# USTC-StarTeam/DR4SR

Hardware: AMD Instinct MI355X
Metric: training sequences/sec, SASRec d=64 L=50 (higher is better)
Workload: dtype f32; 1 GPU; SASRec on amazon-toys-shaped synthetic rows (BASELINE configs[1]): N=11925, L=50, d=64, 2 layers, 2 heads, FFN 128, dropout 0.50, B=256 rows/GPU/step, toys histogram (10.9% valid) seqlen; global_batch=256, seq_len=50, parallelism=dp1, hip_graph=True, steps_per_graph=30

## Files before the change

dr4sr_amd/_lib.py:

```python
from __future__ import annotations

import ctypes as C
import os

_HERE = os.path.dirname(os.path.abspath(__file__))
LIB_PATH = os.environ.get("DR4SR_LIB_PATH") or os.path.join(_HERE, "csrc", "libdr4sr_hip.so")

ABI_VERSION = 10
COMM_ID_BYTES = 128
GRAD_TAIL = 4
STATE_WORDS = 16
STATE_STEP, STATE_T, STATE_NVALID, STATE_RNGSTEP = 0, 1, 2, 3
POOL_NONE, POOL_ORIGIN, POOL_LAST, POOL_MEAN = 0, 1, 2, 3
SITE_EMB, SITE_ATTN, SITE_PROJ, SITE_ACT, SITE_FFN = 0, 1, 2, 3, 4
OPT_ADAM, OPT_SGD, OPT_ADAGRAD, OPT_RMSPROP = 0, 1, 2, 3


def check_ids(idx, n_items: int, what: str = "index"):
    import torch
    if idx is None or idx.numel() == 0:
        return
    bad = torch.zeros(1, dtype=torch.int32, device=idx.device)
    t = idx.contiguous()
    check(load().dr4sr_check_ids(ptr(t), t.numel(), int(n_items), ptr(bad), cur_stream()), "dr4sr_check_ids")
# ... 21 lines not shown
    if n == "rmsprop":
        return OPT_RMSPROP, (0.9, 0.99), 1e-8, float(weight_decay)
    if n == "sparse_adam":
        raise RuntimeError("SparseAdam does not support dense gradients, please consider Adam instead")
    return OPT_ADAM, (0.9, 0.999), 1e-8, 0.0

KERNEL_IDS = {"prep": 0, "embed_fwd": 1, "qkv_fwd": 2, "attn_fwd": 3, "post_fwd": 4, "score": 5, "transpose": 6,
              "post_bwd": 7, "attn_bwd": 8, "qkv_bwd": 9, "embed_bwd": 10, "wgrad": 11, "adam": 12, "zero_grads": 13,
              "embqkv_fwd": 14, "post_mid": 15, "qkv_embed_bwd": 16, "wgrad_fused": 17}

FMLP_KERNEL_IDS = {"filter_fwd": 0, "ffn_fwd": 1, "ffn_bwd": 2, "filter_bwd": 3, "wgrad": 4}

_f32p = C.c_void_p
_i64p = C.c_void_p


_PLAN_BUFFERS = [("seed", C.c_uint64),
                 ("params", _f32p), ("grads", _f32p), ("adam_m", _f32p), ("adam_v", _f32p),
                 ("n_params", C.c_int64)]
_PLAN_WORKSPACE = [("sample_neg", C.c_int32),
                   ("workspace", C.c_void_p), ("workspace_bytes", C.c_int64),
                   ("state", C.c_void_p)]
_PLAN_OPTIMIZER = [("lr", C.c_float), ("beta1", C.c_float), ("beta2", C.c_float), ("adam_eps", C.c_float), ("weight_decay", C.c_float)]
_PLAN_PERM_LOG = [("perm", _i64p), ("n_perm", C.c_int64), ("perm_stride", C.c_int64), ("perm_offset", C.c_int64),
                  ("perm_counter", C.c_void_p),
                  ("loss_log", _f32p)]


def _i32(*names):
    return [(n, C.c_int32) for n in names]


def _ptrs(*names):
    return [(n, _i64p) for n in names]


class SasrecPlan(C.Structure):
    _fields_ = (_i32("abi_version", "B", "L", "D", "H", "F", "n_layer", "n_items") + [("ln_eps", C.c_float), ("p_drop", C.c_float)]
                + _PLAN_BUFFERS + _ptrs("in_item_id", "item_id", "seqlen", "rows", "neg_item") + _PLAN_WORKSPACE + _PLAN_OPTIMIZER
                + _PLAN_PERM_LOG + _i32("expected_tokens", "optimizer"))


class MetaWeighting(C.Structure):
    _fields_ = [("phi", _f32p), ("gumbel", _f32p), ("user_id", _i64p), ("gate_in", C.c_void_p), ("gate_out", C.c_void_p),
                ("weight_out", _f32p), ("tau", C.c_float)]


class FmlpPlan(C.Structure):
    _fields_ = (_i32("abi_version", "B", "L", "D", "F", "n_layer", "n_items") + [("ln_eps", C.c_float), ("p_drop", C.c_float)]
                + _PLAN_BUFFERS + _ptrs("in_item_id", "item_id", "rows", "neg_item") + _PLAN_WORKSPACE + _PLAN_OPTIMIZER
                + _i32("optimizer") + _PLAN_PERM_LOG)


class GruPlan(C.Structure):
    _fields_ = (_i32("abi_version", "B", "L", "D", "H", "n_layer", "n_items") + [("p_drop", C.c_float)]
                + _PLAN_BUFFERS + _ptrs("in_item_id", "item_id", "seqlen", "rows", "neg_item") + _PLAN_WORKSPACE + _PLAN_OPTIMIZER
                + _i32("optimizer") + _PLAN_PERM_LOG)


class RegenPlan(C.Structure):
    _fields_ = [
        ("abi_version", C.c_int32),
        ("n_rows", C.c_int32), ("K", C.c_int32), ("max_len", C.c_int32),
        ("D", C.c_int32), ("H", C.c_int32), ("F", C.c_int32), ("n_layer", C.c_int32),
        ("ln_eps", C.c_float),
        ("params", _f32p),
        ("n_params", C.c_int64),
    ]


REGEN_TENSORS = 70
REGEN_SCORE_TENSORS = 98

_PLANP = C.POINTER(SasrecPlan)
_FPLANP = C.POINTER(FmlpPlan)
_GPLANP = C.POINTER(GruPlan)
_RPLANP = C.POINTER(RegenPlan)

SYMBOLS = {
    "dr4sr_abi_version": (C.c_int, []),
    "dr4sr_sasrec_plan_sizeof": (C.c_int, []),
    "dr4sr_sasrec_param_layout": (C.c_int64, [C.c_int32, C.c_int32, C.c_int32, C.c_int32, C.c_int32, C.c_void_p]),
    "dr4sr_sasrec_workspace_bytes": (C.c_int64, [_PLANP]),
    "dr4sr_sasrec_at_scale": (C.c_int, [C.c_void_p]),
    "dr4sr_sasrec_fwd_bwd": (C.c_int, [_PLANP, C.c_void_p]),
    "dr4sr_adam_step": (C.c_int, [_PLANP, C.c_void_p]),
    "dr4sr_sasrec_fwd_bwd_weighted": (C.c_int, [_PLANP, C.c_void_p, C.c_void_p]),
    "dr4sr_sasrec_fwd_bwd_weighted_prepared": (C.c_int, [_PLANP, C.c_void_p, C.c_void_p]),
    "dr4sr_sasrec_train_step": (C.c_int, [_PLANP, C.c_void_p]),
    "dr4sr_sasrec_train_steps": (C.c_int, [_PLANP, C.c_int32, C.c_void_p]),
    "dr4sr_sasrec_fwd_bwd_prepared": (C.c_int, [_PLANP, C.c_void_p]),
    "dr4sr_adam_step_prepare_next": (C.c_int, [_PLANP, C.c_void_p]),
    "dr4sr_sasrec_grad_buckets": (C.c_int, [_PLANP, C.POINTER(C.c_int64)]),
    "dr4sr_sasrec_fwd_bwd_phase": (C.c_int, [_PLANP, C.c_int32, C.c_int32, C.c_void_p]),
    "dr4sr_sasrec_encode": (C.c_int, [_PLANP, C.c_int32, C.c_int32, _f32p, C.c_void_p]),
    "dr4sr_sasrec_encode_bwd": (C.c_int, [_PLANP, C.c_int32, C.c_int32, _f32p, C.c_void_p]),
    "dr4sr_select_rows": (C.c_int, [_i64p, C.c_int64, _i64p, C.c_int32, C.c_int64, C.c_int64, C.c_void_p, C.c_void_p]),
    "dr4sr_embed_gather_posadd": (C.c_int, [_f32p, _f32p, _i64p, _f32p, C.c_int64, C.c_int32, C.c_int32, C.c_int32, C.c_void_p]),
    "dr4sr_score_bce_fwd": (C.c_int, [_f32p, _f32p, _i64p, _i64p, _f32p, _f32p, _f32p, _f32p, C.c_int64, C.c_int32, C.c_int32, C.c_void_p]),
    "dr4sr_score_bce_bwd": (C.c_int, [_f32p, _f32p, _i64p, _i64p, _f32p, _f32p, _f32p, _f32p, C.c_int64, C.c_int32, C.c_int32, C.c_void_p]),
    "dr4sr_score_bpr_fwd": (C.c_int, [_f32p, _f32p, _i64p, _i64p, _f32p, _f32p, _f32p, _f32p, C.c_int64, C.c_int32, C.c_int32, C.c_void_p]),
    "dr4sr_score_bpr_bwd": (C.c_int, [_f32p, _f32p, _i64p, _i64p, _f32p, _f32p, _f32p, _f32p, C.c_int64, C.c_int32, C.c_int32, C.c_void_p]),
    "dr4sr_loss_from_scores_fwd": (C.c_int, [_f32p, _f32p, C.c_int64, C.c_int32, C.c_int32, _f32p, _f32p, C.c_void_p]),
    "dr4sr_loss_from_scores_bwd": (C.c_int, [_f32p, _f32p, C.c_int64, C.c_int32, C.c_int32, _f32p, _f32p, _f32p, _f32p, C.c_void_p]),
    "dr4sr_neg_sample": (C.c_int, [_i64p, C.c_int64, C.c_int32, C.c_uint64, C.c_uint32, C.c_void_p]),
    "dr4sr_neg_sample_dev": (C.c_int, [_i64p, C.c_int64, C.c_int32, C.c_uint64, C.c_void_p, C.c_void_p]),
    "dr4sr_dropout_mask": (C.c_int, [_f32p, C.c_int64, C.c_float, C.c_uint64, C.c_uint32, C.c_uint32, C.c_void_p]),
    "dr4sr_fmlp_plan_sizeof": (C.c_int, []),
    "dr4sr_fmlp_param_layout": (C.c_int64, [C.c_int32, C.c_int32, C.c_int32, C.c_int32, C.c_int32, C.c_void_p]),
    "dr4sr_fmlp_workspace_bytes": (C.c_int64, [_FPLANP]),
    "dr4sr_fmlp_fwd_bwd": (C.c_int, [_FPLANP, C.c_void_p]),
    "dr4sr_fmlp_train_step": (C.c_int, [_FPLANP, C.c_void_p]),
    "dr4sr_fmlp_encode": (C.c_int, [_FPLANP, C.c_int32, _f32p, C.c_void_p]),
    "dr4sr_fmlp_encode_bwd": (C.c_int, [_FPLANP, C.c_int32, _f32p, C.c_void_p]),
    "dr4sr_gru4rec_plan_sizeof": (C.c_int, []),
    "dr4sr_gru4rec_param_layout": (C.c_int64, [C.c_int32, C.c_int32, C.c_int32, C.c_int32, C.c_void_p]),
    "dr4sr_gru4rec_workspace_bytes": (C.c_int64, [_GPLANP]),
    "dr4sr_gru4rec_uses_cooperative": (C.c_int, [C.c_int32, C.c_int32]),
    "dr4sr_gru4rec_uses_wavefront": (C.c_int, [C.c_int32, C.c_int32, C.c_int32, C.c_int32]),
    "dr4sr_gru4rec_fwd_bwd": (C.c_int, [_GPLANP, C.c_void_p]),
    "dr4sr_gru4rec_train_step": (C.c_int, [_GPLANP, C.c_void_p]),
    "dr4sr_gru4rec_encode": (C.c_int, [_GPLANP, C.c_int32, C.c_int32, _f32p, C.c_void_p]),
    "dr4sr_gru4rec_encode_bwd": (C.c_int, [_GPLANP, C.c_int32, C.c_int32, _f32p, C.c_void_p]),
    "dr4sr_adam_flat": (C.c_int, [_f32p, _f32p, _f32p, _f32p, C.c_int64, C.c_void_p, C.c_float, C.c_float, C.c_float, C.c_float, C.c_float, C.c_void_p]),
    "dr4sr_reload_env": (C.c_int, []),
    "dr4sr_build_flags": (C.c_int, []),
    "dr4sr_sasrec_launch_kernel": (C.c_int, [_PLANP, C.c_int32, C.c_int32, C.c_void_p]),
    "dr4sr_sasrec_launch_kernel_weighted": (C.c_int, [_PLANP, C.c_void_p, C.c_int32, C.c_int32, C.c_void_p]),
    "dr4sr_gru4rec_launch_kernel": (C.c_int, [_GPLANP, C.c_int32, C.c_int32, C.c_void_p]),
    "dr4sr_fmlp_launch_kernel": (C.c_int, [_FPLANP, C.c_int32, C.c_int32, C.c_void_p]),
    "dr4sr_meta_param_count": (C.c_int64, [C.c_int32]),
    "dr4sr_meta_select_workspace_floats": (C.c_int64, [C.c_int64]),
    "dr4sr_meta_select_workspace_floats_d": (C.c_int64, [C.c_int64, C.c_int32]),
    "dr4sr_meta_select_fwd": (C.c_int, [_f32p, _f32p, _f32p, C.c_uint64, C.c_uint32, C.c_void_p, C.c_float, _i64p, _i64p, C.c_int64, C.c_int32,
                                        C.c_int32, C.c_void_p, C.c_void_p, _f32p, C.c_void_p]),
    "dr4sr_meta_select_bwd": (C.c_int, [_f32p, _f32p, _f32p, C.c_uint64, C.c_uint32, C.c_void_p, C.c_float, _i64p, _i64p, C.c_int64, C.c_int32,
                                        C.c_int32, C.c_void_p, _f32p, _f32p, _f32p, _f32p, _f32p, C.c_void_p]),
    "dr4sr_meta_select_fwd_d": (C.c_int, [_f32p, _f32p, _f32p, C.c_uint64, C.c_uint32, C.c_void_p, C.c_float, _i64p, _i64p, C.c_int64, C.c_int32,
                                          C.c_int32, C.c_void_p, C.c_void_p, _f32p, C.c_void_p]),
    "dr4sr_meta_select_bwd_d": (C.c_int, [_f32p, _f32p, _f32p, C.c_uint64, C.c_uint32, C.c_void_p, C.c_float, _i64p, _i64p, C.c_int64, C.c_int32,
                                          C.c_int32, C.c_void_p, _f32p, _f32p, _f32p, _f32p, _f32p, C.c_void_p]),
    "dr4sr_fd_step_size": (C.c_int, [_f32p, _f32p, C.c_int64, C.c_float, _f32p, C.c_void_p]),
    "dr4sr_fd_step_size_scratch_floats": (C.c_int64, []),
    "dr4sr_fd_step_size_ws": (C.c_int, [_f32p, _f32p, C.c_int64, C.c_float, _f32p, _f32p, C.c_void_p]),
    "dr4sr_fd_shift": (C.c_int, [_f32p, _f32p, _f32p, _f32p, C.c_float, C.c_int64, C.c_void_p]),
    "dr4sr_fd_neumann": (C.c_int, [_f32p, _f32p, _f32p, _f32p, _f32p, _f32p, _f32p, C.c_float, C.c_int64, C.c_void_p]),
    "dr4sr_fd_diff": (C.c_int, [_f32p, _f32p, _f32p, _f32p, _f32p, _f32p, C.c_float, C.c_int64, C.c_void_p]),
    "dr4sr_fd_diff4": (C.c_int, [_f32p, _f32p, _f32p, _f32p, _f32p, _f32p, _f32p, C.c_float, C.c_int64, C.c_void_p]),
    "dr4sr_scale_by": (C.c_int, [_f32p, _f32p, _f32p, C.c_int64, C.c_void_p]),
    "dr4sr_meta_opt_step": (C.c_int, [C.c_int32, _f32p, _f32p, _f32p, _f32p, C.c_int32, C.c_float, C.c_float, C.c_float, C.c_float, C.c_float,
                                      C.c_float, C.c_void_p, _f32p, C.c_void_p]),
    "dr4sr_meta_sgd_step": (C.c_int, [_f32p, _f32p, _f32p, C.c_int32, C.c_float, C.c_float, C.c_float, C.c_float, C.c_void_p,
                                      _f32p, C.c_void_p]),
    "dr4sr_cl_augment": (C.c_int, [_i64p, _i64p, _i64p, _i64p, C.c_int32, C.c_int32, C.c_int32, C.c_double, C.c_double, C.c_double,
                                   C.c_int64, C.c_uint64, C.c_uint32, C.c_void_p]),
    "dr4sr_cl_augment_dev": (C.c_int, [_i64p, _i64p, _i64p, _i64p, C.c_int32, C.c_int32, C.c_int32, C.c_double, C.c_double, C.c_double,
                                       C.c_int64, C.c_uint64, C.c_void_p, C.c_uint32, C.c_void_p]),
    "dr4sr_cl_augment2_dev": (C.c_int, [_i64p, _i64p, _i64p, _i64p, _i64p, _i64p, C.c_int32, C.c_int32, C.c_int32, C.c_double, C.c_double,
                                        C.c_double, C.c_int64, C.c_uint64, C.c_void_p, C.c_uint32, C.c_void_p]),
    "dr4sr_cl_augment2_rows_dev": (C.c_int, [_i64p, _i64p, _i64p, _i64p, _i64p, _i64p, _i64p, C.c_int32, C.c_int32, C.c_int32, C.c_double,
                                             C.c_double, C.c_double, C.c_int64, C.c_uint64, C.c_void_p, C.c_uint32, C.c_void_p]),
    "dr4sr_cl_prepare": (C.c_int, [_i64p, C.c_int32, C.c_void_p, _f32p, _f32p, C.c_int64, C.c_void_p]),
    "dr4sr_cl_prepare_rows": (C.c_int, [_i64p, _i64p, C.c_int32, C.c_void_p, _f32p, _f32p, C.c_int64, C.c_void_p]),
    "dr4sr_cl_prepare_rows_step": (C.c_int, [_i64p, _i64p, C.c_int32, C.c_void_p, _f32p, _f32p, C.c_int64, C.c_void_p, C.c_int32, C.c_void_p]),
    "dr4sr_infonce_bwd_scaled": (C.c_int, [_f32p, _f32p, C.c_void_p, C.c_int32, C.c_int32, C.c_float, _f32p, _f32p, _f32p, C.c_float, C.c_int32,
                                           _f32p, _f32p, C.c_void_p]),
# ... 125 lines not shown
```

dr4sr_amd/csrc/attn_tile.h:

```cpp
#pragma once
#include "common.h"
#include "kernels.h"

#define TSTAMP(i, thr) do { if (P.stamps && blockIdx.x == 0 && threadIdx.x == (thr)) P.stamps[i] = __builtin_amdgcn_s_memtime(); } while (0)
namespace tattn {

constexpr int WR = 80;
constexpr int QR0 = 64;
constexpr int MT = WR / 16;

template <int D>
struct Lds {
    static constexpr int LD = D + 4;
    static constexpr int floats = 2 * WR * LD + 16 * LD + 64 + 32 + 2 * WR + 8;
    float *Kw, *Vw, *Qs, *st, *rd; int2* tok; unsigned* pad;
    __device__ __forceinline__ explicit Lds(float* base) {
        Kw = base; Vw = Kw + WR * LD; Qs = Vw + WR * LD;
        st = Qs + 16 * LD;
        rd = st + 64;
        tok = reinterpret_cast<int2*>(rd + 32);
        pad = reinterpret_cast<unsigned*>(tok + WR);
    }
};

// ... 53 lines not shown
    __device__ __forceinline__ void issue(const TileAttnArgs& A, const int t0, const int T, const int r_lo = 0, const int r_hi = WR) {
        const int wb = t0 - QR0, lo = max(0, t0 - (A.L - 1)), hi = min(T, t0 + 16);
        tw = make_int2(0x7fffffff, 0);
        if ((int)threadIdx.x >= r_lo && (int)threadIdx.x < r_hi) {
            const int tk = wb + (int)threadIdx.x;
            if (tk >= lo && tk < hi) tw = A.tok[tk];
        }
#pragma unroll
        for (int q = 0; q < PER; ++q) {
            const int f = threadIdx.x + 256 * q, r = f / C4, c4 = f % C4, tk = wb + r;
            v[q] = make_float4(0.f, 0.f, 0.f, 0.f);
            if (r >= r_lo && r < r_hi && tk >= lo && tk < hi) v[q] = ld4(A.qkv + (size_t)tk * 3 * D + D + 4 * c4);
        }
        if constexpr (WITH_Q) {
#pragma unroll
            for (int q = 0; q < QPER; ++q) {
                const int f = threadIdx.x + 256 * q, r = f / (D / 4), c4 = f % (D / 4);
                qv[q] = make_float4(0.f, 0.f, 0.f, 0.f);
                if (t0 + r < T) qv[q] = ld4(A.qkv + (size_t)(t0 + r) * 3 * D + 4 * c4);
            }
        }
        sv = make_float2(0.f, 0.f);
        if constexpr (WITH_STAT) {
            if (threadIdx.x < 32) {
                const int i = threadIdx.x >> 1;
                if (t0 + i < T) sv = *reinterpret_cast<const float2*>(A.stat + ((size_t)(t0 + i) * 2 + (threadIdx.x & 1)) * 2);
            }
        }
    }
    __device__ __forceinline__ void commit(const Lds<D>& S, const int r_lo = 0, const int r_hi = WR) const {
        if ((int)threadIdx.x >= r_lo && (int)threadIdx.x < r_hi) S.tok[threadIdx.x] = tw;
        if (threadIdx.x < 128) {
            const unsigned long long bal = __ballot(((tw.y >> 30) & 1) != 0);
            if (threadIdx.x == 0) {
#pragma unroll
                for (int jt = 0; jt < 4; ++jt)
                    if (16 * jt >= r_lo && 16 * jt < r_hi) S.pad[jt] = (unsigned)(bal >> (16 * jt)) & 0xffffu;
            }
            if (threadIdx.x == 64 && 64 >= r_lo && 64 < r_hi) S.pad[4] = (unsigned)bal & 0xffffu;
        }
#pragma unroll
        for (int q = 0; q < PER; ++q) {
            const int f = threadIdx.x + 256 * q, r = f / C4, c4 = f % C4;
            if (r >= r_lo && r < r_hi) st4((4 * c4 < D ? S.Kw + r * LD + 4 * c4 : S.Vw + r * LD + 4 * c4 - D), v[q]);
        }
        if constexpr (WITH_Q) {
#pragma unroll
            for (int q = 0; q < QPER; ++q) {
                const int f = threadIdx.x + 256 * q, r = f / (D / 4), c4 = f % (D / 4);
                st4(S.Qs + r * LD + 4 * c4, qv[q]);
            }
        }
        if constexpr (WITH_STAT) {
            if (threadIdx.x < 32) {
                const int i = threadIdx.x >> 1, h = threadIdx.x & 1;
                S.st[(h * 16 + i) * 2] = sv.x; S.st[(h * 16 + i) * 2 + 1] = sv.y;
            }
        }
    }
};

constexpr int NEAR0 = WR - 32;
template <int D>
__device__ __forceinline__ void far_rows_if_needed(const TileAttnArgs& A, const Lds<D>& S, const int t0, const int T) {
    if (!(A.on & 4) || S.tok[QR0].x >= t0 - 16) return;
    Stage<D, false, false> st;
    st.issue(A, t0, T, 0, NEAR0);
    st.commit(S, 0, NEAR0);
    lds_barrier();
}

struct Keep { uint32_t lo, hi; };
__device__ __forceinline__ int2 own_word(const TileAttnArgs& A, const int t0, const int T) {
    const int tq = t0 + (int)(threadIdx.x & 15);
    return tq < T ? A.tok[tq] : make_int2(0x7fffffff, 0);
}
__device__ __forceinline__ Keep own_keep(const PostArgs& P, const int2 mq, const int t0, const int T) {
    Keep k{0xffffffffu, 0xffffffffu};
    if (P.training && P.p > 0.f) {
        const int tq = t0 + (int)(threadIdx.x & 15), h = (threadIdx.x >> 6) & 1, i = tq < T ? tq - mq.x : -1;
        const RngKey rk = make_rng(P.seed, (uint32_t)P.state[DR4SR_STATE_RNGSTEP], P.p);
        keep_bits(rk, DR4SR_SITE_ATTN + 4 * P.layer, ((uint64_t)((mq.y & 0xfffff) * 2 + h) * 64 + i) * 64, i, k.lo, k.hi);
    }
    return k;
}

template <int D, bool KEEP_QS>
struct FwdPre { Stage<D, KEEP_QS, false> st; int2 mq_g; float qf[D / 8]; uint32_t klo, khi; };
template <int D, bool KEEP_QS>
__device__ __forceinline__ void fwd_issue(const PostArgs& P, const int t0, const int T, FwdPre<D, KEEP_QS>& F) {
    constexpr int DH = D / 2;
    const TileAttnArgs& A = P.at;
    const int h = (threadIdx.x >> 6) & 1;
    F.mq_g = own_word(A, t0, T);
    if constexpr (!KEEP_QS) frag_g<DH>(F.qf, A.qkv + h * DH, 3 * D, t0, T);
    F.st.issue(A, t0, T, (A.on & 4) ? NEAR0 : 0, WR);
}
template <int D, bool KEEP_QS>
__device__ __forceinline__ void fwd_stage(const PostArgs& P, const int t0, const int T, float* base, FwdPre<D, KEEP_QS>& F) {
    const TileAttnArgs& A = P.at;
    const Lds<D> S(base);
    const int r_lo = (A.on & 4) ? NEAR0 : 0;
    TSTAMP(27, 0);
    __builtin_amdgcn_sched_barrier(0);
    const Keep k0 = own_keep(P, F.mq_g, t0, T);
    F.klo = k0.lo; F.khi = k0.hi;
    __builtin_amdgcn_sched_barrier(0);
    TSTAMP(28, 0);
    F.st.commit(S, r_lo, WR);
    TSTAMP(8, 0);
    lds_barrier();
    far_rows_if_needed<D>(A, S, t0, T);
    TSTAMP(9, 0);
}
template <int D, bool KEEP_QS>
__device__ __forceinline__ Keep fwd_compute(const PostArgs& P, const int t0, const int T, float* R0, const int ldr, float* base, FwdPre<D, KEEP_QS>& F) {
    constexpr int DH = D / 2, LD = D + 4, H = 2;
    const TileAttnArgs& A = P.at;
    const Lds<D> S(base);
    const int lane = threadIdx.x & 63, w = threadIdx.x >> 6, h = w & 1, half = w >> 1, i16 = lane & 15, g = lane >> 4;
    const uint32_t klo_ = F.klo, khi_ = F.khi;
    float qf[DH / 4];
    if constexpr (!KEEP_QS) {
#pragma unroll
        for (int c = 0; c < DH / 4; ++c) qf[c] = F.qf[c];
    }
    if constexpr (KEEP_QS) frag<DH>(qf, S.Qs, LD, 0, h * DH);
    const int tq = t0 + i16, wb = t0 - QR0;
    const int2 mq = S.tok[QR0 + i16];
    const bool qok = tq < T;
    const int qs = mq.x;
    const int jt_lo = (S.tok[QR0].x - wb) >> 4;
    const float scale = 1.0f / sqrtf((float)DH);
    f32x4 s[MT];
    float m = -INFINITY;
#pragma unroll
    for (int jt = 0; jt < MT; ++jt) {
        s[jt] = (f32x4){0.f, 0.f, 0.f, 0.f};
        if (jt >= jt_lo) {
            float kf[DH / 4];
            frag<DH>(kf, S.Kw, LD, jt * 16, h * DH);
            s[jt] = mma_rows<DH>(kf, qf);
            const unsigned pw = S.pad[jt] >> (4 * g);
#pragma unroll
            for (int r = 0; r < 4; ++r) {
                const int tk = wb + jt * 16 + 4 * g + r;
                const bool ok = qok && tk >= qs && tk <= tq && !((pw >> r) & 1u);
                const float v = ok ? s[jt][r] * scale : -INFINITY;
                s[jt][r] = v;
                m = fmaxf(m, v);
            }
        }
    }
    TSTAMP(10, 0);
    m = xg_max(m);
    float sum = 0.f;
#pragma unroll
    for (int jt = 0; jt < MT; ++jt)
        if (jt >= jt_lo)
#pragma unroll
            for (int r = 0; r < 4; ++r) { const float e = __expf(s[jt][r] - m); s[jt][r] = e; sum += e; }
    sum = xg_sum(sum);
    const float inv = 1.0f / sum;
    if (half == 0 && g == 0) {
        if (qok) { float* st = A.stat + ((size_t)tq * H + h) * 2; st[0] = m; st[1] = inv; }
        if constexpr (KEEP_QS) { S.st[(h * 16 + i16) * 2] = m; S.st[(h * 16 + i16) * 2 + 1] = inv; }
// ... 154 lines not shown
```

dr4sr_amd/csrc/embed.hip:

```cpp
#include "common.h"
#include "kernels.h"
#include <cstdlib>

template <int D>
__global__ __launch_bounds__(256) void k_embed_dense(const float* __restrict__ E, const float* __restrict__ P,
                                                         const int64_t* __restrict__ idx, float* __restrict__ out,
                                                         int64_t ntok, int L, int n_items) {
    constexpr int LPT = D / 4;
    constexpr int TPB = 256 / LPT;
    const int sub = threadIdx.x / LPT, c = (threadIdx.x % LPT) * 4;
    for (int64_t t = (int64_t)blockIdx.x * TPB + sub; t < ntok; t += (int64_t)gridDim.x * TPB) {
        int64_t id = idx[t];
        id = id < 0 ? 0 : (id >= n_items ? n_items - 1 : id);
        const int l = (int)(t % L);
        const float4 e = ld4(E + id * D + c);
        const float4 p = ld4(P + (size_t)l * D + c);
        const f32x4 v = {e.x + p.x, e.y + p.y, e.z + p.z, e.w + p.w};
        __builtin_nontemporal_store(v, reinterpret_cast<f32x4*>(out + t * D + c));
    }
}

extern "C" int dr4sr_embed_gather_posadd(const float* E, const float* P, const int64_t* idx, float* out,
                                         int64_t B, int32_t L, int32_t D, int32_t n_items, void* stream) {
    if (!E || !P || !idx || !out || B < 0 || L <= 0 || n_items <= 0) return DR4SR_E_ARG;
    if (D != 64 && D != 128) return DR4SR_E_SHAPE;
    const int64_t ntok = B * L;
    if (ntok == 0) return 0;
    const int tpb = 256 / (D / 4);
    int64_t blocks = (ntok + tpb - 1) / tpb;
    const int64_t cap = DR4SR_XENV("DR4SR_GATHER_BLOCKS") ? atoll(DR4SR_XENV("DR4SR_GATHER_BLOCKS")) : 65536;
    if (blocks > cap) blocks = cap;
    hipStream_t s = (hipStream_t)stream;
    if (D == 64) hipLaunchKernelGGL(k_embed_dense<64>, dim3((unsigned)blocks), dim3(256), 0, s, E, P, idx, out, ntok, L, n_items);
    else hipLaunchKernelGGL(k_embed_dense<128>, dim3((unsigned)blocks), dim3(256), 0, s, E, P, idx, out, ntok, L, n_items);
    return DR4SR_LAUNCH_CHECK();
}

__global__ __launch_bounds__(256) void k_check_ids(const int64_t* __restrict__ idx, int64_t n, int n_items, int* __restrict__ bad) {
    int c = 0;
    for (int64_t i = (int64_t)blockIdx.x * 256 + threadIdx.x; i < n; i += (int64_t)gridDim.x * 256) {
        const int64_t id = idx[i];
        c += (id < 0 || id >= n_items) ? 1 : 0;
    }
    c = (int)wave_sum((float)c);
    if ((threadIdx.x & 63) == 0 && c) atomicAdd(bad, c);
}
extern "C" int dr4sr_check_ids(const int64_t* idx, int64_t n, int32_t n_items, int32_t* bad_count, void* stream) {
    if (!idx || !bad_count || n < 0 || n_items <= 0) return DR4SR_E_ARG;
    if (n == 0) return 0;
    int64_t blocks = (n + 255) / 256;
    if (blocks > 1024) blocks = 1024;
    hipLaunchKernelGGL(k_check_ids, dim3((unsigned)blocks), dim3(256), 0, (hipStream_t)stream, idx, n, n_items, bad_count);
    return DR4SR_LAUNCH_CHECK();
}

#include "prep_body.h"
__global__ __launch_bounds__(1024) void k_prep(const PrepArgs P, float* __restrict__ zero, int64_t zero_n4) {
    if (blockIdx.x > 0) {
        for (int64_t i = (int64_t)(blockIdx.x - 1) * 1024 + threadIdx.x; i < zero_n4; i += (int64_t)(gridDim.x - 1) * 1024)
            st4(zero + 4 * i, make_float4(0.f, 0.f, 0.f, 0.f));
        return;
    }
    __shared__ unsigned long long part[1024];
    prep_body<1024>(P, part);
}

static int launch_prep_sel(const int64_t* seqlen, const int64_t* rows, int* cu, int* state, int B, int L, int bump_rng, float* zero,
                           int64_t zero_floats, const PermSel& sel, int* tile_seq, int* seq_class, hipStream_t s) {
    const int64_t n4 = zero ? zero_floats / 4 : 0;
    int zb = (int)((n4 + 1023) / 1024);
    if (zb > 255) zb = 255;
    const PrepArgs P{seqlen, rows, cu, state, B, L, bump_rng, sel, tile_seq, seq_class, nullptr};
    hipLaunchKernelGGL(k_prep, dim3(1 + zb), dim3(1024), 0, s, P, zero, n4);
    return DR4SR_LAUNCH_CHECK();
}
int launch_prep_raw(const int64_t* seqlen, const int64_t* rows, int* cu, int* state, int B, int L, int bump_rng, float* zero,
                    int64_t zero_floats, hipStream_t s) {
    return launch_prep_sel(seqlen, rows, cu, state, B, L, bump_rng, zero, zero_floats, PermSel{nullptr, 0, 0, 0, nullptr}, nullptr, nullptr, s);
}
int launch_prep_raw_hints(const int64_t* seqlen, const int64_t* rows, int* cu, int* state, int B, int L, int bump_rng, float* zero,
                          int64_t zero_floats, int* tile_seq, const PermSel& sel, hipStream_t s) {
    return launch_prep_sel(seqlen, rows, cu, state, B, L, bump_rng, zero, zero_floats, sel, tile_seq, nullptr, s);
}
int make_prep_args(const dr4sr_sasrec_plan* p, const Workspace& ws, int bump_rng, PrepArgs* out) {
    PermSel sel{nullptr, 0, 0, 0, nullptr};
    if (p->perm && bump_rng) {
        if (!p->rows || !p->perm_counter || p->n_perm <= 0) return DR4SR_E_ARG;
        sel = PermSel{p->perm, p->n_perm, p->perm_stride, p->perm_offset, p->perm_counter};
    }
    *out = PrepArgs{p->seqlen, p->rows, ws.cu, p->state, p->B, p->L, bump_rng, sel, ws.tile_seq, (ws.attn_split && !attn_wave_on(p, ws)) ? ws.seq_class : nullptr, ws.len_buf};
    return 0;
}
int launch_prep(const dr4sr_sasrec_plan* p, const Workspace& ws, int bump_rng, int zero_grads, hipStream_t s) {
    PrepArgs P;
    const int rc = make_prep_args(p, ws, bump_rng, &P);
    if (rc) return rc;
    return launch_prep_sel(p->seqlen, p->rows, ws.cu, p->state, p->B, p->L, bump_rng, zero_grads ? p->grads : nullptr,
                           ws.n_params + DR4SR_GRAD_TAIL, P.sel, ws.tile_seq, P.seq_class, s);
}


template <int D>
__global__ __launch_bounds__(256) void k_embed_fwd(const float* __restrict__ E, const float* __restrict__ P,
                                                   const int64_t* __restrict__ idx, const int64_t* __restrict__ rows,
                                                   const int* __restrict__ cu, float* __restrict__ X, int B, int L,
                                                   int n_items, const int* __restrict__ state, uint64_t seed, float p,
                                                   int training) {
    constexpr int LPT = D / 4, TPB = 256 / LPT;
    const int T = state[DR4SR_STATE_T];
    const int t = blockIdx.x * TPB + threadIdx.x / LPT, c = (threadIdx.x % LPT) * 4;
    if (t >= T) return;
    const int b = find_seq(cu, B, t), pos = t - cu[b];
    const int64_t row = rows ? rows[b] : b;
    int64_t id = idx[row * L + pos];
    id = id < 0 ? 0 : (id >= n_items ? n_items - 1 : id);
    float4 o = ld4(E + id * D + c);
    if (P) {
        const float4 pe = ld4(P + (size_t)pos * D + c);
        o = make_float4(o.x + pe.x, o.y + pe.y, o.z + pe.z, o.w + pe.w);
    }
    if (training && p > 0.f) {
        const RngKey rk = make_rng(seed, (uint32_t)state[DR4SR_STATE_RNGSTEP], p);
        const float4 m = drop4(rk, DR4SR_SITE_EMB, ((uint64_t)b * L + pos) * D + c);
        o.x *= m.x; o.y *= m.y; o.z *= m.z; o.w *= m.w;
    }
    st4(X + (size_t)t * D + c, o);
}

int launch_embed_fwd_raw(const float* E, const float* P, const int64_t* idx, const int64_t* rows, const int* cu, float* X, int B,
                         int L, int D, int n_items, const int* state, uint64_t seed, float p, int training, hipStream_t s) {
    dim3 grid(((int64_t)B * L + (256 / (D / 4)) - 1) / (256 / (D / 4))), blk(256);
    if (D == 64) hipLaunchKernelGGL(k_embed_fwd<64>, grid, blk, 0, s, E, P, idx, rows, cu, X, B, L, n_items, state, seed, p, training);
    else hipLaunchKernelGGL(k_embed_fwd<128>, grid, blk, 0, s, E, P, idx, rows, cu, X, B, L, n_items, state, seed, p, training);
    return DR4SR_LAUNCH_CHECK();
}
int launch_embed_fwd(const dr4sr_sasrec_plan* p, const Workspace& ws, int training, hipStream_t s) {
    return launch_embed_fwd_raw(p->params + ws.off[0], p->params + ws.off[1], p->in_item_id, p->rows, ws.cu, ws.X[0], p->B, p->L,
                                p->D, p->n_items, p->state, p->seed, p->p_drop, training, s);
}

template <int D>
__global__ __launch_bounds__(256) void k_embed_bwd(const float* __restrict__ dX, const int64_t* __restrict__ idx,
                                                   const int64_t* __restrict__ rows, const int* __restrict__ cu,
                                                   float* __restrict__ dE, float* __restrict__ dP, int B, int L,
                                                   int n_items, const int* __restrict__ state, uint64_t seed, float p,
                                                   int training) {
    constexpr int LPT = D / 4, TPB = 256 / LPT;
    __shared__ float accP[64 * D];
    const int T = state[DR4SR_STATE_T], t0 = blockIdx.x * 64;
    if (t0 >= T) return;
    if (dP) for (int i = threadIdx.x; i < L * D; i += 256) accP[i] = 0.f;
    __syncthreads();
    const int c = (threadIdx.x % LPT) * 4;
    const bool dodrop = training && p > 0.f;
    const RngKey rk = make_rng(seed, (uint32_t)state[DR4SR_STATE_RNGSTEP], p);
    for (int t = t0 + threadIdx.x / LPT; t < min(T, t0 + 64); t += TPB) {
        const int b = find_seq(cu, B, t), pos = t - cu[b];
        const int64_t row = rows ? rows[b] : b;
        float4 g = ld4(dX + (size_t)t * D + c);
        if (dodrop) {
            const float4 m = drop4(rk, DR4SR_SITE_EMB, ((uint64_t)b * L + pos) * D + c);
            g.x *= m.x; g.y *= m.y; g.z *= m.z; g.w *= m.w;
        }
        if (dP) {
            float* a = accP + pos * D + c;
            atomicAdd(a, g.x); atomicAdd(a + 1, g.y); atomicAdd(a + 2, g.z); atomicAdd(a + 3, g.w);
        }
        const int64_t id = idx[row * L + pos];
        if (id > 0 && id < n_items) {
            float* d = dE + id * D + c;
            unsafeAtomicAdd(d, g.x); unsafeAtomicAdd(d + 1, g.y); unsafeAtomicAdd(d + 2, g.z); unsafeAtomicAdd(d + 3, g.w);
        }
    }
    if (dP) {
        __syncthreads();
        for (int i = threadIdx.x; i < L * D; i += 256) {
            const float v = accP[i];
            if (v != 0.f) unsafeAtomicAdd(dP + i, v);
        }
    }
}
// ... 127 lines not shown
```

dr4sr_amd/csrc/kernels.h:

```cpp
#pragma once
#include <hip/hip_runtime.h>
#include <stdint.h>
#include "../../include/dr4sr_hip.h"
#include "../../include/dr4sr_hip_hooks.h"
#include "prep_body.h"

#define DR4SR_MAX_LAYERS 8

struct LayerWs {
    float* qkv;
    float* ctx;
    float* attn_st;
    unsigned* attn_keep;
    float* u1;
    float* y;
    float* st1;
    float* a;
    float* h;
    float* u2;
    float* st2;
    float* df;
    float* da;
    float* du1;
    float* dout;
    float* dqkv;
    unsigned short* row_keep;
};

struct Workspace {
    int64_t off[2 + 12 * DR4SR_MAX_LAYERS];
    int64_t n_params;
    int Tmax;
    int* cu;
    bool scale, attn_split;
    bool attn_tile_sa;
    int* len_buf;
    int* seq_class;
    float* attn_rd;
    int* tile_seq;
    float* X[DR4SR_MAX_LAYERS + 1];
    float* dX[DR4SR_MAX_LAYERS + 1];
    float* dctx;
    int4* de_rec;
    int* idx32;
    int2* tok;
    int4* de_ent;
    unsigned char* de_off;
    bool det;
    bool scale_wg, det_lat; float* det_kv; int64_t det_kv_layer;
    float* det_part; float* det_ln; float* det_dp; int64_t det_stride;
    float* wfrag;
    unsigned short* wsplit;
    int64_t wsplit_E;
    float* wT;
    int64_t wT_stride;
    float* score_part;
    float* ln_part;
    LayerWs layer[DR4SR_MAX_LAYERS];
    int64_t bytes;
};

enum { P_IN_W = 0, P_IN_B, P_OUT_W, P_OUT_B, P_W1, P_B1, P_W2, P_B2, P_LN1_W, P_LN1_B, P_LN2_W, P_LN2_B };
static inline int64_t poff(const Workspace& ws, int layer, int j) { return ws.off[2 + 12 * layer + j]; }
int latency_tmax();
static inline bool at_scale(int Tmax) { return Tmax > latency_tmax(); }
constexpr int DR4SR_SCALE_TOKENS = 7168, DR4SR_ATTN_SPLIT_TOKENS = 14336;
constexpr int DR4SR_SCALE_TOKENS_SHORT = 10240, DR4SR_SCALE_TOKENS_LONG = 6144;
constexpr int DR4SR_SCALE_TOKENS_SHORT_WAVE = 7680;
bool attn_tile_capable(const dr4sr_sasrec_plan* p);
bool tile_xcd_order(const dr4sr_sasrec_plan* p, const Workspace& ws);
__host__ __device__ inline int xcd_per(const int tiles, const int BM) {
    const int q = BM < 64 ? 64 / BM : 1, per = (tiles + 7) >> 3;
    return (per + q - 1) / q * q;
}
static inline int xcd_grid(int tiles, int BM) { return 8 * xcd_per(tiles, BM); }
#if defined(__HIPCC__)
__device__ __forceinline__ int xcd_tile(const int T, const int BM, const int on) {
    if (!on) return (int)blockIdx.x;
    const int nt = (T + BM - 1) / BM, per = xcd_per(nt, BM), x = (int)blockIdx.x & 7, j = (int)blockIdx.x >> 3;
    return (j < per && x * per + j < nt) ? x * per + j : nt;
}
#endif

struct TileAttnArgs {
    const float* qkv; float* dqkv; float* ctx; float* stat; const int2* tok; int L;
    unsigned* keep;
    int on;
    float* kv_part;
};
struct alignas(16) PostArgs {
    const float* ctx; const float* x;
    const float* out_w; const float* out_b; const float* ln1_w; const float* ln1_b;
    const float* w1; const float* b1; const float* w2; const float* b2; const float* ln2_w; const float* ln2_b;
    float* u1; float* y; float* st1; float* a; float* h; float* u2; float* st2; float* z;
    const float* dz; const float* w2T; const float* w1T; const float* out_wT;
    float* df; float* da; float* du1; float* dout; float* dctx;
    float* rd; int n_head;
    float* ln_part;
    const int* state; uint64_t seed; float p; float eps; int layer; int training;
    uint32_t sP, sA, sF;
    unsigned long long* stamps;
    const float* nx_in_w; const float* nx_in_b; float* nx_qkv;
    const float* up_dqkv; const float* up_in_w; const float* up_du1;
    const float* up_kv_part;
    TileAttnArgs at;
    int xcd;
    float* nx_dqkv_zero;
    float* dn_dqkv_zero;
    int wt_attn;
    unsigned short* row_keep;
    const unsigned short* sp;
};

struct EmbQkvArgs {
    const float* E; const float* P; const int64_t* idx; const int64_t* rows; const int* cu; const int* tile_seq; float* X;
    const float* W; const float* bias; float* QKV; const int* state;
    int B, L, n_items, training; uint64_t seed; float p;
    int* idx32;
    int2* tok; float* dqkv_zero;
    int xcd;
    int wf_layers;
    const unsigned short* sp;
};
struct QkvEmbBwdArgs {
    const float* dQKV; const float* W; const float* dU1; const int64_t* idx; const int64_t* rows; const int* cu; const int* tile_seq;
    float* dE; float* dP; const int* state; int B, L, n_items, training; uint64_t seed; float p;
    float* gout;
    const float* kv_part; const int2* tok;
    const unsigned short* sp;
};

struct ScoreTileArgs {
    const float* E; float* dE; const int64_t* target; const int64_t* rows; const int* cu; const int* tile_seq; int64_t* neg_item; float* part;
    int sample_neg, n_items, B, L;
    int4* rec;
    int4* ent; unsigned char* off; const int* idx32; int logG;
    const float* phi; const float* gumbel; const int64_t* user_id; const unsigned long long* gate_in; unsigned long long* gate_out;
    float* w_out; float inv_tau; uint64_t meta_seed;
};

struct WgradJob {
    const float* G; int ldg; int gcol;
    const float* X; int ldx;
    float* dW; float* db;
    int ldw;
};
#define DR4SR_DET_MAX_SPLITS 320
#define DR4SR_WGRAD_MAX_JOBS 12
struct WgradArgs {
    WgradJob job[DR4SR_WGRAD_MAX_JOBS * DR4SR_MAX_LAYERS];
    int jobs_per_layer;
    const int* state; uint64_t seed; float p; int training;
    const float* ln_part; int64_t ln_layer_stride; float* grads; int64_t o_ln1_w; int64_t layer_stride;
    const float* score_part; float* tail; int B; int D;
    int score_tiles;
    int ln_tile_rows;
    int ln_rows[DR4SR_MAX_LAYERS];
    int qeb_plane;
    int layer0;
    int bf16x3;
    int xcd;
    const float* fc_dm; int64_t fc_o_cw; int fc_L;
    const float* sc_g; const int64_t* sc_idx; const int64_t* sc_rows; const int* sc_tile_seq; const int* cu;
    float* sc_dE; float* sc_dP; int sc_L; int sc_n_items;
    const int4* ow_ent; const unsigned char* ow_off;
    int ow_on; const int4* ow_rec; const int* ow_idx32; const float* ow_z; int ow_logG, ow_planes, ow_rpo;
    float* det; int det_stride; float* det_ln; float* det_dp;
};

bool wave_tiles(const dr4sr_sasrec_plan* p, const Workspace& ws);
bool wt_bwd_on();
int launch_wt_post_fwd(const PostArgs& A, int Tmax, hipStream_t s);
int launch_wt_post_bwd(const PostArgs& A, int Tmax, hipStream_t s);

int launch_wt_post_mid(const PostArgs& A, const ScoreTileArgs& S, int Tmax, hipStream_t s);
int launch_wt_embqkv_fwd(const EmbQkvArgs& A, int Tmax, hipStream_t s);
int launch_wt_qkv_embed_bwd(const QkvEmbBwdArgs& A, int Tmax, hipStream_t s);

int ffn_tile_rows(int Tmax);
int launch_ffn_fwd(const PostArgs& A, int Tmax, hipStream_t s);
int launch_ffn_bwd(const PostArgs& A, int Tmax, hipStream_t s);
int launch_fmlp_wgrad(const WgradArgs& A, int Tmax, int n_layer, hipStream_t s);
int launch_table_owner64(const int* state, const int4* rec, const int* idx32, const float* z, const float* g, float* dE, int n_items, hipStream_t s);
int launch_adam_flat(float* P, float* G, float* M, float* V, int64_t n, int* state, float lr, float b1, float b2, float eps, float wd, hipStream_t s,
                     float* loss_log = nullptr, const int* log_index = nullptr, const PrepArgs* next = nullptr, int opt = DR4SR_OPT_ADAM);

int carve_workspace(const dr4sr_sasrec_plan* p, Workspace* ws);

int launch_prep(const dr4sr_sasrec_plan* p, const Workspace& ws, int bump_rng, int zero_grads, hipStream_t s);
int make_prep_args(const dr4sr_sasrec_plan* p, const Workspace& ws, int bump_rng, PrepArgs* out);
int launch_embed_fwd(const dr4sr_sasrec_plan* p, const Workspace& ws, int training, hipStream_t s);
int launch_embed_bwd(const dr4sr_sasrec_plan* p, const Workspace& ws, int training, hipStream_t s);
int launch_unpack(const dr4sr_sasrec_plan* p, const Workspace& ws, const float* X, float* out, int mode, hipStream_t s);
int launch_pack(const dr4sr_sasrec_plan* p, const Workspace& ws, const float* dout, float* dX, int mode, hipStream_t s);

int launch_transpose_weights(const dr4sr_sasrec_plan* p, const Workspace& ws, hipStream_t s);
bool tile_bf3(const dr4sr_sasrec_plan* p, const Workspace& ws);
int launch_wsplit(const dr4sr_sasrec_plan* p, const Workspace& ws, hipStream_t s);
int launch_wfrag_write(const dr4sr_sasrec_plan* p, const Workspace& ws, hipStream_t s);
bool wfrag_img_on(const dr4sr_sasrec_plan* p, const Workspace& ws);
int launch_wsplit_raw(const float* params, unsigned short* img, int64_t o_in, int64_t o_out, int64_t o_w1, int64_t o_w2, int64_t layer_stride,
                      int E, int D, int F, int n_layer, hipStream_t s);
int launch_embqkv_fwd(const dr4sr_sasrec_plan* p, const Workspace& ws, int training, hipStream_t s);
int launch_qkv_embed_bwd(const dr4sr_sasrec_plan* p, const Workspace& ws, int training, hipStream_t s);
int launch_post_mid(const dr4sr_sasrec_plan* p, const Workspace& ws, int training, hipStream_t s, const dr4sr_meta_weighting* mw = nullptr);
int launch_qkv_fwd(const dr4sr_sasrec_plan* p, const Workspace& ws, int layer, hipStream_t s);
int launch_post_fwd(const dr4sr_sasrec_plan* p, const Workspace& ws, int layer, int training, hipStream_t s);
int launch_post_bwd(const dr4sr_sasrec_plan* p, const Workspace& ws, int layer, int training, hipStream_t s);
int launch_qkv_bwd(const dr4sr_sasrec_plan* p, const Workspace& ws, int layer, hipStream_t s);
int launch_wgrad(const dr4sr_sasrec_plan* p, const Workspace& ws, int training, int with_score, hipStream_t s, bool qeb = false,
                 bool meta = false, int l_lo = 0, int l_hi = -1, int table = -1);
bool wgrad_table_jobs(const dr4sr_sasrec_plan* p, const Workspace& ws);
bool attn_in_tile(const dr4sr_sasrec_plan* p, const Workspace& ws);
bool attn_wave_on(const dr4sr_sasrec_plan* p, const Workspace& ws);
bool attn_fold_fwd(const dr4sr_sasrec_plan* p, const Workspace& ws);
PostArgs make_post_args(const dr4sr_sasrec_plan* p, const Workspace& ws, int layer, int training);
int launch_attn_tile_fwd(const dr4sr_sasrec_plan* p, const Workspace& ws, int layer, int training, hipStream_t s);
int launch_attn_tile_bwd(const dr4sr_sasrec_plan* p, const Workspace& ws, int layer, int training, hipStream_t s);
bool qeb_in_wgrad(const Workspace& ws);

int launch_attn_fwd(const dr4sr_sasrec_plan* p, const Workspace& ws, int layer, int training, hipStream_t s);
int launch_attn_bwd(const dr4sr_sasrec_plan* p, const Workspace& ws, int layer, int training, hipStream_t s);

struct GruWaveArgs {
    const float* gi1; const float* whh[2]; const float* wih2; const int* cu;
    float* r[2]; float* z[2]; float* n[2]; float* ghn[2]; float* hprev[2]; float* hout[2];
    const float* dhout; float* dgi[2]; float* dgh[2];
};
int launch_prep_raw(const int64_t* seqlen, const int64_t* rows, int* cu, int* state, int B, int L, int bump_rng, float* zero,
                    int64_t zero_floats, hipStream_t s);
int launch_prep_raw_hints(const int64_t* seqlen, const int64_t* rows, int* cu, int* state, int B, int L, int bump_rng, float* zero,
                          int64_t zero_floats, int* tile_seq, const PermSel& sel, hipStream_t s);
int launch_embed_fwd_raw(const float* E, const float* P, const int64_t* idx, const int64_t* rows, const int* cu, float* X, int B,
                         int L, int D, int n_items, const int* state, uint64_t seed, float p, int training, hipStream_t s);
int launch_embed_bwd_raw(const float* dX, const int64_t* idx, const int64_t* rows, const int* cu, float* dE, float* dP, int B, int L,
                         int D, int n_items, const int* state, uint64_t seed, float p, int training, hipStream_t s);
int launch_unpack_raw(const float* X, const int* cu, float* out, int B, int L, int D, int last, hipStream_t s);
int launch_pack_raw(const float* dout, const int* cu, float* dX, int B, int L, int D, int last, hipStream_t s);
int launch_score_packed_raw(const float* Z, const float* E, float* dE, float* dZ, const int64_t* target, const int64_t* rows,
                            const int* cu, int64_t* neg_item, int sample_neg, float* part, const int* state, uint64_t seed,
                            int n_items, int B, int L, int D, hipStream_t s, int4* rec = nullptr);

int launch_attn2_fwd(const dr4sr_sasrec_plan* p, const Workspace& ws, int layer, int training, hipStream_t s);
int launch_attn2_bwd(const dr4sr_sasrec_plan* p, const Workspace& ws, int layer, int training, hipStream_t s);

int launch_score_packed(const dr4sr_sasrec_plan* p, const Workspace& ws, hipStream_t s);
int launch_adam(const dr4sr_sasrec_plan* p, hipStream_t s, const PrepArgs* next = nullptr);
```

dr4sr_amd/csrc/linear.hip:

```cpp
#include "common.h"
#include "kernels.h"
#include <cstdlib>
#define STAMP(i) do { if (A.stamps && blockIdx.x == 0 && threadIdx.x == 0) A.stamps[i] = __builtin_amdgcn_s_memtime(); } while (0)

extern __shared__ __attribute__((aligned(16))) float smem[];

__global__ __launch_bounds__(256) void k_transpose(const float* __restrict__ params, float* __restrict__ wT,
                                                   int64_t o_in, int64_t o_out, int64_t o_w1, int64_t o_w2,
                                                   int64_t layer_stride, int64_t wT_stride, int D, int F) {
    const int m = blockIdx.y, layer = blockIdx.z;
    const float* src;
    float* dst = wT + layer * wT_stride;
    int R, C;
    if (m == 0) { src = params + o_in + layer * layer_stride; R = 3 * D; C = D; }
    else if (m == 1) { src = params + o_out + layer * layer_stride; R = D; C = D; dst += 3 * D * D; }
    else if (m == 2) { src = params + o_w1 + layer * layer_stride; R = F; C = D; dst += 4 * D * D; }
    else { src = params + o_w2 + layer * layer_stride; R = D; C = F; dst += 4 * D * D + D * F; }
    for (int i = blockIdx.x * 256 + threadIdx.x; i < R * C; i += gridDim.x * 256) {
        const int r = i / C, c = i % C;
        dst[c * R + r] = src[i];
    }
}

int launch_transpose_weights(const dr4sr_sasrec_plan* p, const Workspace& ws, hipStream_t s) {
// ... 187 lines not shown
template <int BM, int D>
__global__ __launch_bounds__(256) void k_embqkv_fwd(const EmbQkvArgs A) {
    constexpr int N = 3 * D, LDA = D + 4, LPT = D / 4, TPB = 256 / LPT;
    if constexpr (BM == 16 && D == 128) { if (A.wf_layers > 0) wfrag_image_write<D>(A); }
    const int T = A.state[DR4SR_STATE_T], t0 = xcd_tile(T, BM, A.xcd) * BM;
    if (t0 >= T) return;
    float* As = smem;
    const int c = (threadIdx.x % LPT) * 4;
    const bool dodrop = A.training && A.p > 0.f;
    const RngKey rk = make_rng(A.seed, (uint32_t)A.state[DR4SR_STATE_RNGSTEP], A.p);
    constexpr bool PFE = BM == 16 && D == 64;
    WFragT<PFE ? D : 16, PFE ? N : 64> f_in;
    if constexpr (PFE) wfrag_load(f_in, A.W, D);
    const int bh = A.tile_seq[t0 >> 4];
#pragma unroll
    for (int r0 = 0; r0 < BM; r0 += TPB) {
        const int r = r0 + threadIdx.x / LPT, t = t0 + r;
        if (r < BM) {
            float4 o = make_float4(0.f, 0.f, 0.f, 0.f);
            if (t < T) {
                const int b = find_seq_from(A.cu, A.B, t, bh), pos = t - A.cu[b];
                const int64_t row = A.rows ? A.rows[b] : b;
                int64_t id = A.idx[row * A.L + pos];
                if (A.idx32 && c == 0) A.idx32[t] = (id > 0 && id < A.n_items) ? (int)id : 0;
                if (A.tok && c == 0) A.tok[t] = make_int2(t - pos, b | ((A.cu[b + 1] - A.cu[b]) << 20) | (id == 0 ? 1 << 30 : 0));
                id = id < 0 ? 0 : (id >= A.n_items ? A.n_items - 1 : id);
                o = ld4(A.E + id * D + c);
                const float4 pe = ld4(A.P + (size_t)pos * D + c);
                o = make_float4(o.x + pe.x, o.y + pe.y, o.z + pe.z, o.w + pe.w);
                if (dodrop) {
                    const float4 m = drop4(rk, DR4SR_SITE_EMB, ((uint64_t)b * A.L + pos) * D + c);
                    o.x *= m.x; o.y *= m.y; o.z *= m.z; o.w *= m.w;
                }
                st4(A.X + (size_t)t * D + c, o);
            }
            st4(As + r * LDA + c, o);
        }
    }
    lds_barrier();
    TileAcc<BM, N> acc;
    tile_zero(acc);
    if constexpr (PFE) tile_mma_frag<BM, D, N>(As, LDA, f_in, acc);
    else tile_gemm<D == 128 && BM == 32, BM, D, N>(As, LDA, A.W, D, false, A.sp, WSplitGeo<D, 128>::E, 0, acc);
    tile_to_global<BM, N>(acc, A.QKV, N, A.bias, t0, T);
    if (A.dqkv_zero) zero_kv_rows<BM, D>(A.dqkv_zero, t0, T);
}

int launch_embqkv_fwd(const dr4sr_sasrec_plan* p, const Workspace& ws, int training, hipStream_t s) {
    const int D = p->D, bm = tile_rows(ws);
    const size_t lds = sizeof(float) * bm * (D + 4);
    dim3 grid((ws.Tmax + bm - 1) / bm), blk(256);
    EmbQkvArgs A;
    A.E = p->params + ws.off[0]; A.P = p->params + ws.off[1]; A.idx = p->in_item_id; A.rows = p->rows; A.cu = ws.cu; A.tile_seq = ws.tile_seq; A.X = ws.X[0];
    A.W = p->params + poff(ws, 0, P_IN_W); A.bias = p->params + poff(ws, 0, P_IN_B); A.QKV = ws.layer[0].qkv; A.state = p->state;
    A.B = p->B; A.L = p->L; A.n_items = p->n_items; A.training = training; A.seed = p->seed; A.p = p->p_drop;
    A.idx32 = de_owner_mode(ws) ? ws.idx32 : nullptr;
    A.sp = wsplit_of(p, ws, 0); A.wf_layers = 0;
    if (wfrag_img_on(p, ws)) { A.sp = reinterpret_cast<const unsigned short*>(ws.wfrag); A.wf_layers = p->n_layer; }
    const bool in_tile = attn_in_tile(p, ws);
    A.tok = (in_tile || ws.attn_tile_sa || attn_wave_on(p, ws)) ? ws.tok : nullptr; A.dqkv_zero = in_tile ? ws.layer[0].dqkv : nullptr;
    A.xcd = tile_xcd_order(p, ws) ? 1 : 0;
    if (A.xcd) grid.x = xcd_grid((int)grid.x, bm);
    if (wave_tiles(p, ws)) return launch_wt_embqkv_fwd(A, ws.Tmax, s);
#define EQ(B_) do { if (D == 64) hipLaunchKernelGGL((k_embqkv_fwd<B_, 64>), grid, blk, lds, s, A); \
                    else hipLaunchKernelGGL((k_embqkv_fwd<B_, 128>), grid, blk, lds, s, A); } while (0)
    BM_DISPATCH(bm, EQ);
#undef EQ
    return DR4SR_LAUNCH_CHECK();
}


struct LnCarry { float4 v; float mean, rstd; uint32_t keep; };
template <int F>
struct RowCarry { LnCarry ln1, ln2; float4 a[F / 64]; uint32_t akeep; };
__host__ __device__ constexpr bool carry_vals(int CARRY) { return CARRY != 0; }
__host__ __device__ constexpr bool carry_bits(int CARRY) { return CARRY == 1 || CARRY == 3; }
__device__ __forceinline__ uint32_t keep_bits4(const float4& m) {
    return (m.x != 0.f ? 1u : 0u) | (m.y != 0.f ? 2u : 0u) | (m.z != 0.f ? 4u : 0u) | (m.w != 0.f ? 8u : 0u);
}
__device__ __forceinline__ float4 keep_factors4(const RngKey& k, uint32_t bits) {
    return make_float4((bits & 1u) ? k.scale : 0.f, (bits & 2u) ? k.scale : 0.f, (bits & 4u) ? k.scale : 0.f, (bits & 8u) ? k.scale : 0.f);
}

template <int BM, int D, bool RES_IN_LDS, bool COPY_LDS, bool CARRY = false, bool KPRE = false>
__device__ __forceinline__ void ln_rowpass(const float* __restrict__ Cs, int ldc, const float* res, int ldres,
                                           const float* __restrict__ lnw, const float* __restrict__ lnb, float eps,
                                           float* __restrict__ U, float* __restrict__ OUT, float* __restrict__ ST,
                                           float* Ls, int ldl, int t0, int T, bool dodrop, const RngKey& rk,
                                           uint32_t site, float4 (*yreg)[D / 64] = nullptr, LnCarry* cy = nullptr) {
    constexpr int NV = D / 64, PASSES = BM / 16;
    static_assert(!CARRY || (NV == 1 && PASSES == 1), "the carried row state is one float4 per thread");
    static_assert(!KPRE || CARRY, "the keep bits arrive in the carried row state");
    const int l16 = threadIdx.x & 15, rsub = threadIdx.x >> 4;
    float4 gam[NV], bet[NV], v[PASSES][NV];
    float mean[PASSES], rstd[PASSES];
#pragma unroll
    for (int j = 0; j < NV; ++j) { gam[j] = ld4(lnw + 4 * l16 + 64 * j); bet[j] = ld4(lnb + 4 * l16 + 64 * j); }
#pragma unroll
    for (int ps = 0; ps < PASSES; ++ps) {
        const int row = ps * 16 + rsub, t = t0 + row;
        const bool ok = t < T;
#pragma unroll
        for (int j = 0; j < NV; ++j) {
            const int c = 4 * l16 + 64 * j;
            float4 o = ld4(Cs + row * ldc + c);
            float4 r = make_float4(0.f, 0.f, 0.f, 0.f);
            if (RES_IN_LDS) r = ld4(res + row * ldres + c);
            else if constexpr (KPRE) r = cy->v;
            else if (ok) r = ld4(res + (size_t)t * ldres + c);
            if (dodrop) {
                float4 m;
                if constexpr (KPRE) m = keep_factors4(rk, cy->keep); else m = drop4(rk, site, (uint64_t)t * D + c);
                o.x *= m.x; o.y *= m.y; o.z *= m.z; o.w *= m.w;
                if constexpr (CARRY && !KPRE) cy->keep = keep_bits4(m);
            }
            v[ps][j] = make_float4(r.x + o.x, r.y + o.y, r.z + o.z, r.w + o.w);
            if (ok) st4(U + (size_t)t * D + c, v[ps][j]);
        }
    }
#pragma unroll
    for (int ps = 0; ps < PASSES; ++ps) ln_stats16<NV>(v[ps], mean[ps], rstd[ps], eps);
    if constexpr (CARRY) { cy->v = v[0][0]; cy->mean = mean[0]; cy->rstd = rstd[0]; }
#pragma unroll
    for (int ps = 0; ps < PASSES; ++ps) {
        const int row = ps * 16 + rsub, t = t0 + row;
        const bool ok = t < T;
#pragma unroll
        for (int j = 0; j < NV; ++j) {
            const int c = 4 * l16 + 64 * j;
            const float m = mean[ps], rs = rstd[ps];
            const float4 yv = make_float4((v[ps][j].x - m) * rs * gam[j].x + bet[j].x, (v[ps][j].y - m) * rs * gam[j].y + bet[j].y,
                                          (v[ps][j].z - m) * rs * gam[j].z + bet[j].z, (v[ps][j].w - m) * rs * gam[j].w + bet[j].w);
            if (ok && OUT) st4(OUT + (size_t)t * D + c, yv);
            if (yreg) yreg[ps][j] = ok ? yv : make_float4(0.f, 0.f, 0.f, 0.f);
            if (COPY_LDS) st4(Ls + row * ldl + c, ok ? yv : make_float4(0.f, 0.f, 0.f, 0.f));
        }
        if (ok && l16 == 0) { ST[2 * (size_t)t] = mean[ps]; ST[2 * (size_t)t + 1] = rstd[ps]; }
    }
}

template <int F>
__device__ __forceinline__ void row_keep_store(const PostArgs& A, const RowCarry<F>& cy, const int t0, const int T) {
    static_assert(F == 128, "16 bits per thread");
    const int t = t0 + (threadIdx.x >> 4);
    if (t < T) A.row_keep[16 * (size_t)t + (threadIdx.x & 15)] = (unsigned short)(cy.ln1.keep | (cy.ln2.keep << 4) | (cy.akeep << 8));
}
__device__ __forceinline__ uint32_t row_keep_word(const RngKey& rk, const uint32_t sP, const uint32_t sF, const uint32_t sA, const bool actdrop, const int t) {
    constexpr int D = 64, F = 128;
    const int l16 = threadIdx.x & 15, pr = l16 >> 1;
    const bool odd = l16 & 1;
    const uint32_t b0 = drop_bits8(rk, odd ? sF : sP, (uint64_t)t * D + 8 * pr);
    const uint32_t b1 = actdrop ? drop_bits8(rk, sA, (uint64_t)t * F + (odd ? 64 : 0) + 8 * pr) : 0xffu;
    const uint32_t own0 = odd ? b0 >> 4 : b0 & 15u, own1 = odd ? b1 >> 4 : b1 & 15u;
    const uint32_t give = odd ? (b0 & 15u) | ((b1 & 15u) << 4) : (b0 >> 4) | (b1 & 0xf0u);
    const uint32_t got = (uint32_t)__shfl_xor((int)give, 1, 64), got0 = got & 15u, got1 = got >> 4;
    return odd ? got0 | (own0 << 4) | (got1 << 8) | (own1 << 12) : own0 | (got0 << 4) | (own1 << 8) | (got1 << 12);
}
template <int BM, int D, int F, bool FFN_ONLY, bool KEEPQ = false, int CARRY = 0, bool KU = false>
__device__ __forceinline__ void post_fwd_body(const PostArgs& A, const int t0, const int T, float4 (*zreg)[D / 64] = nullptr,
                                              tattn::Keep* keep_out = nullptr, RowCarry<F>* cy = nullptr) {
    constexpr int LD = D + 4, LF = F + 4, NVF = F / 64, PASSES = BM / 16;
    float* R0 = smem;
    float* R1 = R0 + BM * LD;
    float* R2 = R1 + BM * LD;
    const int l16 = threadIdx.x & 15, rsub = threadIdx.x >> 4;
    const bool dodrop = A.training && A.p > 0.f;
    const RngKey rk = make_rng(A.seed, (uint32_t)A.state[DR4SR_STATE_RNGSTEP], A.p);
    const uint32_t sP = A.sP, sA = A.sA, sF = A.sF;
    const bool actdrop = dodrop && sA != 0xffffffffu;

    constexpr bool PF = BM == 16 && !FFN_ONLY;
    WFragT<PF ? D : 16, PF ? D : 64> f_out;
    WFragT<PF ? D : 16, PF ? F : 64> f_w1;
    WFragT<PF ? F : 16, PF ? D : 64> f_w2;
    WFragT<PF ? D : 16, PF ? 3 * D : 64> f_nx;
    STAMP(0);
    static_assert(!KU || (BM == 16 && D == 64 && F == 128 && !FFN_ONLY && CARRY != 0), "one row, one float4, 16 keep bits per thread");
    auto keep_upfront = [&]() {
        if constexpr (KU) {
            const uint32_t w = row_keep_word(rk, sP, sF, sA, actdrop, t0 + rsub);
            cy->ln1.keep = w & 15u; cy->ln2.keep = (w >> 4) & 15u; cy->akeep = w >> 8;
        }
    };
    if constexpr (KU) {
        const int t = t0 + rsub;
        cy->ln1.v = t < T ? ld4(A.x + (size_t)t * D + 4 * l16) : make_float4(0.f, 0.f, 0.f, 0.f);
        __builtin_amdgcn_sched_barrier(0);
    }
    if (FFN_ONLY) {
        load_tile_bm<BM, D>(R1, LD, A.x, D, t0, T);
    } else {
        constexpr bool AT = BM == 16 && (D == 64 || D == 128);
        bool at_on = false;
        if constexpr (AT) at_on = A.at.on != 0;
        if (!at_on) load_tile_bm<BM, D>(R0, LD, A.ctx, D, t0, T);
        tattn::FwdPre<AT ? D : 64, KEEPQ> att_pre;
#ifdef DR4SR_WFRAG_UPFRONT
        constexpr bool SPREAD = false;
#else
        constexpr bool SPREAD = AT && PF;
#endif
        constexpr bool KU_EARLY = KU && SPREAD;
        if constexpr (SPREAD) {
            if (at_on) {
                tattn::fwd_issue<D, KEEPQ>(A, t0, T, att_pre);
                __builtin_amdgcn_sched_barrier(0);
                { if constexpr (D == 128) wfrag_load_img(f_out, reinterpret_cast<const float*>(A.sp) + WSplitGeo<D, F>::OUT); else wfrag_load(f_out, A.out_w, D); }
                __builtin_amdgcn_sched_barrier(0);
                if constexpr (KU_EARLY) { keep_upfront(); __builtin_amdgcn_sched_barrier(0); }
                tattn::fwd_stage<D, KEEPQ>(A, t0, T, smem + att_lds_off(D, F), att_pre);
                __builtin_amdgcn_sched_barrier(0);
                { if constexpr (D == 128) wfrag_load_img(f_w1, reinterpret_cast<const float*>(A.sp) + WSplitGeo<D, F>::W1); else wfrag_load(f_w1, A.w1, D); }
                { if constexpr (D == 128) wfrag_load_img(f_w2, reinterpret_cast<const float*>(A.sp) + WSplitGeo<D, F>::W2); else wfrag_load(f_w2, A.w2, F); }
                __builtin_amdgcn_sched_barrier(0);
                const tattn::Keep k = tattn::fwd_compute<D, KEEPQ>(A, t0, T, R0, LD, smem + att_lds_off(D, F), att_pre);
                if (keep_out) *keep_out = k;
                __builtin_amdgcn_sched_barrier(0);
                if (A.nx_qkv) { if constexpr (D == 128) wfrag_load_img(f_nx, reinterpret_cast<const float*>(A.sp) + WSplitGeo<D, F>::E); else wfrag_load(f_nx, A.nx_in_w, D); }
            } else {
                { if constexpr (D == 128) wfrag_load_img(f_out, reinterpret_cast<const float*>(A.sp) + WSplitGeo<D, F>::OUT); else wfrag_load(f_out, A.out_w, D); }
                { if constexpr (D == 128) wfrag_load_img(f_w1, reinterpret_cast<const float*>(A.sp) + WSplitGeo<D, F>::W1); else wfrag_load(f_w1, A.w1, D); }
                { if constexpr (D == 128) wfrag_load_img(f_w2, reinterpret_cast<const float*>(A.sp) + WSplitGeo<D, F>::W2); else wfrag_load(f_w2, A.w2, F); }
                if (A.nx_qkv) { if constexpr (D == 128) wfrag_load_img(f_nx, reinterpret_cast<const float*>(A.sp) + WSplitGeo<D, F>::E); else wfrag_load(f_nx, A.nx_in_w, D); }
                if constexpr (KU_EARLY) keep_upfront();
            }
        } else {
            constexpr bool EARLY = D == 128;
            if constexpr (AT && EARLY) { if (at_on) { tattn::fwd_issue<D, KEEPQ>(A, t0, T, att_pre); __builtin_amdgcn_sched_barrier(0); } }
            if constexpr (PF) {
                { if constexpr (D == 128) wfrag_load_img(f_out, reinterpret_cast<const float*>(A.sp) + WSplitGeo<D, F>::OUT); else wfrag_load(f_out, A.out_w, D); }
                { if constexpr (D == 128) wfrag_load_img(f_w1, reinterpret_cast<const float*>(A.sp) + WSplitGeo<D, F>::W1); else wfrag_load(f_w1, A.w1, D); }
                { if constexpr (D == 128) wfrag_load_img(f_w2, reinterpret_cast<const float*>(A.sp) + WSplitGeo<D, F>::W2); else wfrag_load(f_w2, A.w2, F); }
                if (A.nx_qkv) { if constexpr (D == 128) wfrag_load_img(f_nx, reinterpret_cast<const float*>(A.sp) + WSplitGeo<D, F>::E); else wfrag_load(f_nx, A.nx_in_w, D); }
            }
            if constexpr (AT) {
                if (at_on) {
                    if constexpr (!EARLY) tattn::fwd_issue<D, KEEPQ>(A, t0, T, att_pre);
                    tattn::fwd_stage<D, KEEPQ>(A, t0, T, smem + att_lds_off(D, F), att_pre);
                    const tattn::Keep k = tattn::fwd_compute<D, KEEPQ>(A, t0, T, R0, LD, smem + att_lds_off(D, F), att_pre);
                    if (keep_out) *keep_out = k;
                }
            }
        }
        lds_barrier(); STAMP(1);
        {
            TileAcc<BM, D> acc;
            tile_zero(acc);
            if constexpr (PF) tile_mma_frag<BM, D, D>(R0, LD, f_out, acc);
            else tile_gemm<BM == 32 && (D == 128 || FFN_ONLY), BM, D, D>(R0, LD, A.out_w, D, false, A.sp, WSplitGeo<D, F>::E, WSplitGeo<D, F>::OUT, acc);
            tile_to_lds<BM, D>(acc, R2, LD, A.out_b);
        }
        lds_barrier(); STAMP(2);
        if constexpr (KU && !KU_EARLY) keep_upfront();
        ln_rowpass<BM, D, false, true, CARRY != 0, KU>(R2, LD, A.x, D, A.ln1_w, A.ln1_b, A.eps, A.u1, A.y, A.st1, R1, LD, t0, T, dodrop, rk, sP, nullptr,
                                                  CARRY ? &cy->ln1 : nullptr);
    }
    lds_barrier(); STAMP(3);
    {
        TileAcc<BM, F> acc;
        tile_zero(acc);
        if constexpr (PF) tile_mma_frag<BM, D, F>(R1, LD, f_w1, acc);
        else tile_gemm<BM == 32 && (D == 128 || FFN_ONLY), BM, D, F>(R1, LD, A.w1, D, false, A.sp, WSplitGeo<D, F>::E, WSplitGeo<D, F>::W1, acc);
        tile_to_lds<BM, F>(acc, R2, LF, A.b1);
    }
    lds_barrier(); STAMP(4);
    {
        float4 av[PASSES][NVF];
#pragma unroll
        for (int ps = 0; ps < PASSES; ++ps)
#pragma unroll
            for (int j = 0; j < NVF; ++j) av[ps][j] = ld4(R2 + (ps * 16 + rsub) * LF + 4 * l16 + 64 * j);
#pragma unroll
        for (int ps = 0; ps < PASSES; ++ps) {
            const int row = ps * 16 + rsub, t = t0 + row;
            const bool ok = t < T;
#pragma unroll
            for (int j = 0; j < NVF; ++j) {
                const int c = 4 * l16 + 64 * j;
                const float4 a4 = av[ps][j];
                float4 h = make_float4(gelu_erf(a4.x), gelu_erf(a4.y), gelu_erf(a4.z), gelu_erf(a4.w));
                if constexpr (CARRY != 0) { cy->a[j] = a4; if (j == 0 && !KU) cy->akeep = 0; }
                if (actdrop) {
                    float4 m;
                    if constexpr (KU) m = keep_factors4(rk, cy->akeep >> (4 * j)); else m = drop4(rk, sA, (uint64_t)t * F + c);
                    h.x *= m.x; h.y *= m.y; h.z *= m.z; h.w *= m.w;
                    if constexpr (CARRY != 0 && !KU) cy->akeep |= keep_bits4(m) << (4 * j);
                }
                if (ok) { st4(A.a + (size_t)t * F + c, a4); st4(A.h + (size_t)t * F + c, h); }
                st4(R2 + row * LF + c, h);
            }
        }
    }
    lds_barrier(); STAMP(5);
    {
        TileAcc<BM, D> acc;
        tile_zero(acc);
        if constexpr (PF) tile_mma_frag<BM, F, D>(R2, LF, f_w2, acc);
        else tile_gemm<BM == 32 && (D == 128 || FFN_ONLY), BM, F, D>(R2, LF, A.w2, F, false, A.sp, WSplitGeo<D, F>::E, WSplitGeo<D, F>::W2, acc);
        tile_to_lds<BM, D>(acc, R0, LD, A.b2);
    }
    lds_barrier(); STAMP(6);
    if (!FFN_ONLY && A.nx_qkv) {
        ln_rowpass<BM, D, true, true, CARRY != 0, KU>(R0, LD, R1, LD, A.ln2_w, A.ln2_b, A.eps, A.u2, A.z, A.st2, R1, LD, t0, T, dodrop, rk, sF, nullptr,
                                                  CARRY ? &cy->ln2 : nullptr);
        if constexpr (CARRY == 2) row_keep_store<F>(A, *cy, t0, T);
        lds_barrier();
        TileAcc<BM, 3 * D> acc;
        tile_zero(acc);
        if constexpr (PF) tile_mma_frag<BM, D, 3 * D>(R1, LD, f_nx, acc);
        else tile_gemm<BM == 32 && (D == 128 || FFN_ONLY), BM, D, 3 * D>(R1, LD, A.nx_in_w, D, false, A.sp ? A.sp + 4 * WSplitGeo<D, F>::E : nullptr, WSplitGeo<D, F>::E, 0, acc);
        tile_to_global<BM, 3 * D>(acc, A.nx_qkv, 3 * D, A.nx_in_b, t0, T);
        if (A.nx_dqkv_zero) zero_kv_rows<BM, D>(A.nx_dqkv_zero, t0, T);
    } else {
        ln_rowpass<BM, D, true, false, CARRY != 0, KU>(R0, LD, R1, LD, A.ln2_w, A.ln2_b, A.eps, A.u2, A.z, A.st2, nullptr, 0, t0, T, dodrop, rk, sF, zreg,
                                                   CARRY ? &cy->ln2 : nullptr);
        if constexpr (CARRY == 2) row_keep_store<F>(A, *cy, t0, T);
    }
    STAMP(15);
}

template <int BM, int D, int F, bool FFN_ONLY, bool KB = false>
__global__ __launch_bounds__(256) void k_post_fwd(const PostArgs A) {
    const int T = A.state[DR4SR_STATE_T], t0 = xcd_tile(T, BM, A.xcd) * BM;
    if (t0 >= T) return;
    if constexpr (KB) {
        RowCarry<F> cy;
        cy.ln1.keep = cy.ln2.keep = cy.akeep = 0;
        post_fwd_body<BM, D, F, FFN_ONLY, false, 2, true>(A, t0, T, nullptr, nullptr, &cy);
    } else post_fwd_body<BM, D, F, FFN_ONLY>(A, t0, T);
}

template <int NV>
__device__ __forceinline__ void flush_affine(const float4 (&dgam)[NV], const float4 (&dbet)[NV], float* scr, float* dst) {
    constexpr int D = 64 * NV;
    const int l16 = threadIdx.x & 15, lane = threadIdx.x & 63, w = threadIdx.x >> 6;
    auto fold = [&](float v) { v += __shfl_xor(v, 16, 64); v += __shfl_xor(v, 32, 64); return v; };
#pragma unroll
    for (int j = 0; j < NV; ++j) {
        const int c = 4 * l16 + 64 * j;
        const float4 a = make_float4(fold(dgam[j].x), fold(dgam[j].y), fold(dgam[j].z), fold(dgam[j].w));
        const float4 b = make_float4(fold(dbet[j].x), fold(dbet[j].y), fold(dbet[j].z), fold(dbet[j].w));
        if (lane < 16) { st4(scr + w * 2 * D + c, a); st4(scr + w * 2 * D + D + c, b); }
    }
    lds_barrier();
    for (int i = threadIdx.x; i < 2 * D; i += 256)
        dst[i] = (scr[i] + scr[2 * D + i]) + (scr[4 * D + i] + scr[6 * D + i]);
    lds_barrier();
}

template <int BM, int D, int SRC, int CARRY = 0>
__device__ __forceinline__ void ln_bwd_rowpass(const float* __restrict__ Gg, const float* La,
                                               const float* Lb, int ldl, const float* __restrict__ Ug,
                                               const float* __restrict__ ST, const float* __restrict__ lnw,
                                               float* __restrict__ DUg, float* DUl, float* __restrict__ DMg,
                                               float* DMl, float4 (&dgam)[D / 64], float4 (&dbet)[D / 64],
                                               int t0, int T, bool dodrop, const RngKey& rk, uint32_t site,
                                               const float4 (*greg)[D / 64] = nullptr, const LnCarry* cy = nullptr) {
    constexpr int NV = D / 64, PASSES = BM / 16;
    static_assert(!CARRY || (NV == 1 && PASSES == 1), "the carried row state is one float4 per thread");
    constexpr bool VALS = carry_vals(CARRY), BITS = carry_bits(CARRY);
    const int l16 = threadIdx.x & 15, rsub = threadIdx.x >> 4;
    float4 gam[NV], g[PASSES][NV], u[PASSES][NV];
    float mean[PASSES], rstd[PASSES];
#pragma unroll
    for (int j = 0; j < NV; ++j) {
        gam[j] = ld4(lnw + 4 * l16 + 64 * j);
        dgam[j] = make_float4(0.f, 0.f, 0.f, 0.f);
        dbet[j] = make_float4(0.f, 0.f, 0.f, 0.f);
    }
#pragma unroll
    for (int ps = 0; ps < PASSES; ++ps) {
        const int row = ps * 16 + rsub, t = t0 + row;
        const bool ok = t < T;
        if constexpr (VALS) { mean[ps] = ok ? cy->mean : 0.f; rstd[ps] = ok ? cy->rstd : 0.f; }
        else { mean[ps] = ok ? ST[2 * (size_t)t] : 0.f; rstd[ps] = ok ? ST[2 * (size_t)t + 1] : 0.f; }
#pragma unroll
        for (int j = 0; j < NV; ++j) {
            const int c = 4 * l16 + 64 * j;
            const float4 z4 = make_float4(0.f, 0.f, 0.f, 0.f);
            if constexpr (VALS) u[ps][j] = ok ? cy->v : z4;
            else u[ps][j] = ok ? ld4(Ug + (size_t)t * D + c) : z4;
            if (SRC == 0) g[ps][j] = ok ? ld4(Gg + (size_t)t * D + c) : z4;
            else if (SRC == 3) g[ps][j] = ok ? greg[ps][j] : z4;
            else {
                const float4 p0 = ld4(La + row * ldl + c);
                float4 p1 = z4;
                if (SRC == 1) p1 = ld4(Lb + row * ldl + c);
                else if (ok) p1 = ld4(Gg + (size_t)t * D + c);
                g[ps][j] = ok ? make_float4(p0.x + p1.x, p0.y + p1.y, p0.z + p1.z, p0.w + p1.w) : z4;
            }
        }
    }
#pragma unroll
    for (int ps = 0; ps < PASSES; ++ps) ln_bwd_row<NV>(g[ps], u[ps], mean[ps], rstd[ps], gam, dgam, dbet);
#pragma unroll
    for (int ps = 0; ps < PASSES; ++ps) {
        const int row = ps * 16 + rsub, t = t0 + row;
// ... 2 lines not shown
        for (int j = 0; j < NV; ++j) {
            const int c = 4 * l16 + 64 * j;
            const float4 du = g[ps][j];
            if (DUg && ok) st4(DUg + (size_t)t * D + c, du);
            if (DUl) st4(DUl + row * ldl + c, du);
            float4 dm = du;
            if (dodrop) {
                float4 m;
                if constexpr (BITS) m = keep_factors4(rk, cy->keep); else m = drop4(rk, site, (uint64_t)t * D + c);
                dm.x *= m.x; dm.y *= m.y; dm.z *= m.z; dm.w *= m.w;
            }
            if (ok) st4(DMg + (size_t)t * D + c, dm);
            st4(DMl + row * ldl + c, dm);
        }
    }
}

template <int BM, int D, int F, bool FFN_ONLY, bool DET = false, int CARRY = 0>
__device__ __forceinline__ void post_bwd_body(const PostArgs& A, const int t0, const int T, const int tile,
                                              const float4 (*dzreg)[D / 64] = nullptr, const tattn::Keep* att_staged = nullptr,
                                              const RowCarry<F>* cy_in = nullptr) {
    constexpr int LD = D + 4, LF = F + 4, NV = D / 64, NVF = F / 64, PASSES = BM / 16;
    float* R1 = smem;
    float* R0 = R1 + BM * LD;
    float* R2 = R0 + BM * LD;
    const int l16 = threadIdx.x & 15, rsub = threadIdx.x >> 4;
    const bool dodrop = A.training && A.p > 0.f;
    const RngKey rk = make_rng(A.seed, (uint32_t)A.state[DR4SR_STATE_RNGSTEP], A.p);
    const uint32_t sP = A.sP, sA = A.sA, sF = A.sF;
    const bool actdrop = dodrop && sA != 0xffffffffu;
    float4 dgam[NV], dbet[NV];
#ifdef DR4SR_BWD_NO_PREFETCH
    constexpr bool PFB = false;
#else
    constexpr bool PFB = BM == 16 && !FFN_ONLY && (D == 64 || D == 128);
#endif
    constexpr bool PF64 = PFB && D == 64, PF128 = PFB && D == 128;
    WFragC<PF64 ? 3 * D : 16, PF64 ? D : 64> fr_up;
    WFragC<PFB ? D : 16, PFB ? F : 64> fr_w2;
    WFragC<PFB ? F : 16, PFB ? D : 64> fr_w1;
    WFragC<PFB ? D : 16, PFB ? D : 64> fr_out;
    constexpr bool AT = BM == 16 && !FFN_ONLY && (D == 64 || D == 128);
    bool at_on = false, at_stage = false;
    tattn::Keep keep{0xffffffffu, 0xffffffffu};
    tattn::Stage<AT ? D : 64, true, true> att_st;
    constexpr int UPQ = AT ? (16 * 3 * D / 4) / 256 : 1;
    float4 updq[UPQ];
    bool up_pre = false;
    RowCarry<F> cy_ld;
    const RowCarry<F>* cy = CARRY >= 2 ? &cy_ld : cy_in;
    if constexpr (AT) {
        at_on = A.at.on != 0;
        at_stage = at_on && !att_staged;
        if (att_staged) keep = *att_staged;
        if (at_on && A.dn_dqkv_zero) zero_kv_rows<BM, D>(A.dn_dqkv_zero, t0, T);
        if (at_stage && A.up_dqkv) {
            up_pre = true;
#pragma unroll
            for (int q = 0; q < UPQ; ++q) {
                const int i = threadIdx.x + 256 * q, row = i / (3 * D / 4), c = (i % (3 * D / 4)) * 4;
                updq[q] = make_float4(0.f, 0.f, 0.f, 0.f);
                if (t0 + row < T) updq[q] = ld4(A.up_dqkv + (size_t)(t0 + row) * 3 * D + c);
            }
            if constexpr (PF64) wfrag_load(fr_up, A.up_in_w, D);
            __builtin_amdgcn_sched_barrier(0);
        }
        if constexpr (CARRY >= 2) {
            static_assert(D == 64 && BM == 16, "one row, one float4 per thread");
            const int t = t0 + rsub, c = 4 * l16;
            const bool ok = t < T;
            const float4 z4 = make_float4(0.f, 0.f, 0.f, 0.f);
            const float2 z2 = make_float2(0.f, 0.f);
            cy_ld.ln2.v = ok ? ld4(A.u2 + (size_t)t * D + c) : z4;
            const float2 s2 = ok ? *reinterpret_cast<const float2*>(A.st2 + 2 * (size_t)t) : z2;
#pragma unroll
            for (int j = 0; j < NVF; ++j) cy_ld.a[j] = ok ? ld4(A.a + (size_t)t * F + c + 64 * j) : z4;
            cy_ld.ln1.v = ok ? ld4(A.u1 + (size_t)t * D + c) : z4;
            const float2 s1 = ok ? *reinterpret_cast<const float2*>(A.st1 + 2 * (size_t)t) : z2;
            cy_ld.ln2.mean = s2.x; cy_ld.ln2.rstd = s2.y; cy_ld.ln1.mean = s1.x; cy_ld.ln1.rstd = s1.y;
            cy_ld.ln1.keep = cy_ld.ln2.keep = cy_ld.akeep = 0;
            if constexpr (CARRY == 3) {
                const uint32_t w = ok ? (uint32_t)A.row_keep[16 * (size_t)t + l16] : 0u;
                cy_ld.ln1.keep = w & 15u; cy_ld.ln2.keep = (w >> 4) & 15u; cy_ld.akeep = w >> 8;
            }
            __builtin_amdgcn_sched_barrier(0);
        }
        if (at_stage) {
            const int2 mq = tattn::own_word(A.at, t0, T);
            att_st.issue(A.at, t0, T, (A.at.on & 4) ? tattn::NEAR0 : 0, tattn::WR);
            __builtin_amdgcn_sched_barrier(0);
            keep = tattn::own_keep(A, mq, t0, T);
            __builtin_amdgcn_sched_barrier(0);
        }
    }
    STAMP(16);
    if constexpr (PFB) { if (!A.up_dqkv) wfrag_load(fr_w2, A.w2, F); else if (PF64 && !up_pre) wfrag_load(fr_up, A.up_in_w, D); }
    auto att_commit = [&]() { if constexpr (AT) { if (at_stage) att_st.commit(tattn::Lds<D>(smem + att_lds_off(D, F)), (A.at.on & 4) ? tattn::NEAR0 : 0, tattn::WR); } };

    if (!FFN_ONLY && A.up_dqkv) {
        constexpr int LQ = 3 * D + 4;
        float* Aq = R0;
        if (AT && up_pre) {
#pragma unroll
            for (int q = 0; q < UPQ; ++q) {
                const int i = threadIdx.x + 256 * q, row = i / (3 * D / 4), c = (i % (3 * D / 4)) * 4;
                st4(Aq + row * LQ + c, updq[q]);
            }
        } else load_tile_bm<BM, 3 * D>(Aq, LQ, A.up_dqkv, 3 * D, t0, T);
        att_commit();
        lds_barrier();
        if constexpr (AT && DET) {
            det_kv_rows<D>(Aq, LQ, const_cast<float*>(A.up_dqkv), A.up_kv_part, A.at.tok, t0, T);
            lds_barrier();
        }
        TileAcc<BM, D> acc;
        tile_zero(acc);
        if constexpr (PF64) { wfrag_load(fr_w2, A.w2, F); tile_mma_frag<BM, 3 * D, D>(Aq, LQ, fr_up, acc); }
        else { tile_gemm<BM == 32 && (D == 128 || FFN_ONLY), BM, 3 * D, D>(Aq, LQ, A.up_in_w, D, true, A.sp ? A.sp + 4 * WSplitGeo<D, F>::E : nullptr, WSplitGeo<D, F>::E, 0, acc); if constexpr (PF128) wfrag_load(fr_w2, A.w2, F); }
        tile_to_lds<BM, D>(acc, R1, LD, nullptr);
        lds_barrier();
        ln_bwd_rowpass<BM, D, 2, CARRY>(A.up_du1, R1, nullptr, LD, A.u2, A.st2, A.ln2_w, nullptr, R1, A.df, R0, dgam, dbet, t0, T, dodrop, rk, sF, nullptr,
                                        CARRY ? &cy->ln2 : nullptr);
    } else if (dzreg) {
        att_commit();
        ln_bwd_rowpass<BM, D, 3, CARRY>(nullptr, nullptr, nullptr, LD, A.u2, A.st2, A.ln2_w, nullptr, R1, A.df, R0, dgam, dbet, t0, T, dodrop, rk, sF, dzreg,
                                        CARRY ? &cy->ln2 : nullptr);
    } else {
        att_commit();
        ln_bwd_rowpass<BM, D, 0, CARRY>(A.dz, nullptr, nullptr, LD, A.u2, A.st2, A.ln2_w, nullptr, R1, A.df, R0, dgam, dbet, t0, T, dodrop, rk, sF, nullptr,
                                        CARRY ? &cy->ln2 : nullptr);
    }
    flush_affine<NV>(dgam, dbet, R2, A.ln_part + (size_t)tile * 4 * D);
    {
        TileAcc<BM, F> acc;
        tile_zero(acc);
        if constexpr (PF64) { wfrag_load(fr_w1, A.w1, D); tile_mma_frag<BM, D, F>(R0, LD, fr_w2, acc); }
        else if constexpr (PF128) { tile_mma_frag<BM, D, F>(R0, LD, fr_w2, acc); wfrag_load(fr_w1, A.w1, D); }
        else tile_gemm<BM == 32 && (D == 128 || FFN_ONLY), BM, D, F>(R0, LD, A.w2, F, true, A.sp, WSplitGeo<D, F>::E, WSplitGeo<D, F>::W2, acc);
        tile_to_lds<BM, F>(acc, R2, LF, nullptr);
    }
    lds_barrier();
#pragma unroll
    for (int ps = 0; ps < PASSES; ++ps) {
        const int row = ps * 16 + rsub, t = t0 + row;
#pragma unroll
        for (int j = 0; j < NVF; ++j) {
            const int c = 4 * l16 + 64 * j;
            float4 d = make_float4(0.f, 0.f, 0.f, 0.f);
            if (t < T) {
                d = ld4(R2 + row * LF + c);
                float4 av;
                if constexpr (carry_vals(CARRY)) av = cy->a[j]; else av = ld4(A.a + (size_t)t * F + c);
                if (actdrop) {
                    float4 m;
                    if constexpr (carry_bits(CARRY)) m = keep_factors4(rk, cy->akeep >> (4 * j)); else m = drop4(rk, sA, (uint64_t)t * F + c);
                    d.x *= m.x; d.y *= m.y; d.z *= m.z; d.w *= m.w;
                }
                d.x *= gelu_erf_grad(av.x); d.y *= gelu_erf_grad(av.y); d.z *= gelu_erf_grad(av.z); d.w *= gelu_erf_grad(av.w);
                st4(A.da + (size_t)t * F + c, d);
            }
            st4(R2 + row * LF + c, d);
        }
    }
    lds_barrier();
    {
        TileAcc<BM, D> acc;
        tile_zero(acc);
        if constexpr (PF64) { wfrag_load(fr_out, A.out_w, D); tile_mma_frag<BM, F, D>(R2, LF, fr_w1, acc); }
        else if constexpr (PF128) { tile_mma_frag<BM, F, D>(R2, LF, fr_w1, acc); wfrag_load(fr_out, A.out_w, D); }
        else tile_gemm<BM == 32 && (D == 128 || FFN_ONLY), BM, F, D>(R2, LF, A.w1, D, true, A.sp, WSplitGeo<D, F>::E, WSplitGeo<D, F>::W1, acc);
        tile_to_lds<BM, D>(acc, R0, LD, nullptr);
    }
    lds_barrier();
    if (FFN_ONLY) {
        constexpr int C4f = D / 4;
// ... 389 lines not shown
#pragma unroll
                        for (int k = 0; k < 4; ++k) { const int j = 4 * sub + k; dh[k] = ((gate >> j) & 1ull) ? (W2[j] - W2[MD + j]) * dzl : 0.f; }
                        dh4[ps] = make_float4(dh[0], dh[1], dh[2], dh[3]);
                    }
                }
            }
#pragma unroll
            for (int ps = 0; ps < PASSES; ++ps) st4(Zs + (ps * 16 + (threadIdx.x >> 4)) * LD + c, dh4[ps]);
            lds_barrier();
            {
                TileAcc<BM, MD> acc;
                tile_zero(acc);
                tile_mma_xw<BM, MD, MD>(Zs, LD, W1, MD, acc);
                tile_to_lds<BM, MD>(acc, Ps, LD, nullptr);
            }
            lds_barrier();
#pragma unroll
            for (int ps = 0; ps < PASSES; ++ps)
                if (on_[ps]) dzw_[ps] = ld4(Ps + (ps * 16 + (threadIdx.x >> 4)) * LD + c);
        }
    }
#pragma unroll
    for (int ps = 0; ps < PASSES; ++ps) {
        float4 dz = make_float4(0.f, 0.f, 0.f, 0.f);
        if (P.ok[ps]) {
            const int t = t0 + ps * 16 + (threadIdx.x >> 4), b = P.b[ps], pos = P.pos[ps], n = P.n[ps];
            const int64_t row = P.row[ps], tgt = P.tgt[ps], ng = P.ng[ps];
            int4 rec = make_int4(0, 0, 0, 0);
            bool on;
            if constexpr (META) on = on_[ps]; else on = tgt > 0 && tgt < S.n_items;
            if (on) {
                const float4 q = zreg[ps][0], ep = P.ep[ps], en = P.en[ps];
                float lt, dpos, dneg, wt = 1.0f;
                float4 dzw = make_float4(0.f, 0.f, 0.f, 0.f);
                if constexpr (META) { lt = lt_[ps]; dpos = dpos_[ps]; dneg = dneg_[ps]; wt = wt_[ps]; dzw = dzw_[ps]; }
                else terms(ps, lt, dpos, dneg);
                if (sub == 0) { lsum += wt * lt; cnt += 1.f; }
                dpos *= wt; dneg *= wt;
                dz = make_float4(dpos * ep.x + dneg * en.x + dzw.x, dpos * ep.y + dneg * en.y + dzw.y, dpos * ep.z + dneg * en.z + dzw.z,
                                 dpos * ep.w + dneg * en.w + dzw.w);
                float* gp = S.dE + tgt * D + c;
                float* gn = S.dE + ng * D + c;
                if (!S.rec) {
                    unsafeAtomicAdd(gp, dpos * q.x); unsafeAtomicAdd(gp + 1, dpos * q.y); unsafeAtomicAdd(gp + 2, dpos * q.z); unsafeAtomicAdd(gp + 3, dpos * q.w);
                    unsafeAtomicAdd(gn, dneg * q.x); unsafeAtomicAdd(gn + 1, dneg * q.y); unsafeAtomicAdd(gn + 2, dneg * q.z); unsafeAtomicAdd(gn + 3, dneg * q.w);
                } else if (sub == 0) {
                    rec = make_int4((int)tgt, (int)ng, __float_as_int(dpos), __float_as_int(dneg));
                }
            }
            if (S.rec && sub == 0) { if (S.ent) lrec[ps * 16 + (threadIdx.x >> 4)] = rec; else S.rec[t] = rec; }
            if (S.ent && sub == 1) reinterpret_cast<int*>(lrec + BM)[ps * 16 + (threadIdx.x >> 4)] = P.idin[ps];
            if (pos == n - 1) {
                for (int l = n + sub; l < S.L; l += LPT) {
                    const int64_t tl = S.target[row * S.L + l];
                    if (S.sample_neg) S.neg_item[(size_t)b * S.L + l] = sample_neg_id(rk, (uint64_t)b * S.L + l, S.n_items);
                    if (tl > 0 && tl < S.n_items) { lsum += 2.0f * 0.69314718055994530942f; cnt += 1.f; }
                }
            }
        }
        dzreg[ps][0] = dz;
    }
    cnt = wave_sum(cnt); lsum = wave_sum(lsum);
    if ((threadIdx.x & 63) == 0) { red[2 * (threadIdx.x >> 6)] = cnt; red[2 * (threadIdx.x >> 6) + 1] = lsum; }
    lds_barrier();
    if (threadIdx.x == 0) {
        S.part[2 * tile] = (red[0] + red[2]) + (red[4] + red[6]);
        S.part[2 * tile + 1] = (red[1] + red[3]) + (red[5] + red[7]);
    }
}

template <int BM, int D, int F, bool META, bool DET = false, bool KU = false>
__device__ __forceinline__ void post_mid_body(const PostArgs& A, const ScoreTileArgs& S) {
    const int T = A.state[DR4SR_STATE_T], bx = xcd_tile(T, BM, A.xcd), t0 = bx * BM;
    if (t0 >= T) return;
    if constexpr (BM != 16) { if (S.ent) tile_sort_init<BM>(S, smem + post_lds_floats(D, F, BM) + 8); }
    if constexpr (D == 64) {
        ScorePre<BM> P;
        if constexpr (BM == 16) score_prefetch<BM>(A, S, t0, T, P);
        float4 zreg[BM / 16][1], dzreg[BM / 16][1];
        PostArgs Af = A;
        if (!S.rec) Af.z = nullptr;
        tattn::Keep keep{0xffffffffu, 0xffffffffu};
        constexpr int CARRY = BM == 16 ? 1 : 0;
        RowCarry<F> cy;
        post_fwd_body<BM, D, F, false, true, CARRY, KU>(Af, t0, T, zreg, &keep, &cy);
        if constexpr (BM != 16) score_prefetch<BM>(A, S, t0, T, P);
        if constexpr (META) lds_barrier();
        score_tile_regs<BM, META>(A, S, t0, T, bx, P, zreg, dzreg, smem + post_lds_floats(D, F, BM), smem);
        if constexpr (BM != 16) { if (S.ent) tile_sort<BM>(S, bx, t0, T, smem + post_lds_floats(D, F, BM) + 8); }
        post_bwd_body<BM, D, F, false, DET, CARRY>(A, t0, T, bx, dzreg, &keep, &cy);
    } else {
        tattn::Keep keep{0xffffffffu, 0xffffffffu};
        post_fwd_body<BM, D, F, false, true>(A, t0, T, nullptr, &keep);
        __syncthreads();
        score_tile<BM, D, META>(A, S, t0, T, bx, smem + post_lds_floats(D, F, BM) + 8);
        if constexpr (BM != 16) { if (S.ent) tile_sort<BM>(S, bx, t0, T, smem + post_lds_floats(D, F, BM) + 8); }
        __syncthreads();
        post_bwd_body<BM, D, F, false, DET>(A, t0, T, bx, nullptr, &keep);
    }
}
template <int BM, int D, int F, bool META, bool DET = false, bool KU = false>
__global__ __launch_bounds__(256) void k_post_mid(const PostArgs A, const ScoreTileArgs S) { post_mid_body<BM, D, F, META, DET, KU>(A, S); }
template <int D, int F>
__global__ __launch_bounds__(256) __attribute__((amdgpu_waves_per_eu(4, 4))) void k_post_mid32(const PostArgs A, const ScoreTileArgs S) {
    post_mid_body<32, D, F, false>(A, S);
}

PostArgs make_post_args(const dr4sr_sasrec_plan* p, const Workspace& ws, int layer, int training) {
    PostArgs A;
    const LayerWs& lw = ws.layer[layer];
    const float* P = p->params;
    A.ctx = lw.ctx; A.x = ws.X[layer];
    A.out_w = P + poff(ws, layer, P_OUT_W); A.out_b = P + poff(ws, layer, P_OUT_B);
    A.ln1_w = P + poff(ws, layer, P_LN1_W); A.ln1_b = P + poff(ws, layer, P_LN1_B);
    A.w1 = P + poff(ws, layer, P_W1); A.b1 = P + poff(ws, layer, P_B1);
    A.w2 = P + poff(ws, layer, P_W2); A.b2 = P + poff(ws, layer, P_B2);
    A.ln2_w = P + poff(ws, layer, P_LN2_W); A.ln2_b = P + poff(ws, layer, P_LN2_B);
    A.u1 = lw.u1; A.y = lw.y; A.st1 = lw.st1; A.a = lw.a; A.h = lw.h; A.u2 = lw.u2; A.st2 = lw.st2; A.z = ws.X[layer + 1];
    A.dz = ws.dX[layer + 1];
    const float* wT = ws.wT + layer * ws.wT_stride;
    const int D = p->D, F = p->F;
    A.out_wT = wT + 3 * D * D; A.w1T = wT + 4 * D * D; A.w2T = wT + 4 * D * D + D * F;
    A.df = lw.df; A.da = lw.da; A.du1 = lw.du1; A.dout = lw.dout; A.dctx = ws.dctx;
    A.rd = p->H == 2 ? ws.attn_rd : nullptr; A.n_head = p->H;
    A.ln_part = ws.ln_part + (size_t)layer * ((ws.Tmax + 15) / 16) * 4 * p->D;
    A.state = p->state; A.seed = p->seed; A.p = p->p_drop; A.eps = p->ln_eps; A.layer = layer; A.training = training;
    A.sP = DR4SR_SITE_PROJ + 4 * layer; A.sA = DR4SR_SITE_ACT + 4 * layer; A.sF = DR4SR_SITE_FFN + 4 * layer;
    A.nx_in_w = A.nx_in_b = nullptr; A.nx_qkv = nullptr; A.up_dqkv = A.up_in_w = A.up_du1 = nullptr;
    if (layer + 1 < p->n_layer && !DR4SR_ENV("DR4SR_NO_FUSE")) {
        A.nx_in_w = P + poff(ws, layer + 1, P_IN_W); A.nx_in_b = P + poff(ws, layer + 1, P_IN_B); A.nx_qkv = ws.layer[layer + 1].qkv;
        A.up_dqkv = ws.layer[layer + 1].dqkv; A.up_in_w = P + poff(ws, layer + 1, P_IN_W); A.up_du1 = ws.layer[layer + 1].du1;
    }
    A.stamps = DR4SR_XENV("DR4SR_STAMPS") ? reinterpret_cast<unsigned long long*>(ws.dctx) : nullptr;
    A.at.on = attn_in_tile(p, ws) ? 1 : 0;
    A.xcd = tile_xcd_order(p, ws) ? 1 : 0;
    const bool near_ok = p->expected_tokens > 0 && p->expected_tokens <= 16 * (int64_t)p->B;
    if (A.at.on && !DR4SR_XENV("DR4SR_ATTN_TILE_FULL") && ((near_ok && p->D == 128) || DR4SR_XENV("DR4SR_ATTN_TILE_NEAR"))) A.at.on |= 4;
    if (A.at.on && DR4SR_ENV("DR4SR_ATTN_TILE_ATOMICS")) A.at.on |= 2;
    A.at.qkv = lw.qkv; A.at.dqkv = lw.dqkv; A.at.ctx = lw.ctx; A.at.stat = lw.attn_st; A.at.tok = ws.tok; A.at.L = p->L; A.at.keep = lw.attn_keep;
    A.wt_attn = attn_fold_fwd(p, ws) ? 1 : 0;
    A.sp = wsplit_of(p, ws, layer);
    if (wfrag_img_on(p, ws)) A.sp = reinterpret_cast<const unsigned short*>(ws.wfrag + (size_t)layer * ws.wT_stride);
    A.at.kv_part = (A.at.on && ws.det_lat && ws.det_kv) ? ws.det_kv + (size_t)layer * ws.det_kv_layer : nullptr;
    A.up_kv_part = (A.at.kv_part && A.up_dqkv) ? ws.det_kv + (size_t)(layer + 1) * ws.det_kv_layer : nullptr;
    A.row_keep = lw.row_keep;
    A.nx_dqkv_zero = (A.at.on && A.nx_qkv) ? ws.layer[layer + 1].dqkv : nullptr;
    A.dn_dqkv_zero = (A.at.on && layer > 0) ? ws.layer[layer - 1].dqkv : nullptr;
    return A;
}

static size_t post_lds(int D, int F, int bm = 64) { return sizeof(float) * post_lds_floats(D, F, bm); }

static bool row_keep_saved(const dr4sr_sasrec_plan* p, const Workspace& ws, const PostArgs& A) {
    return A.training && p->p_drop > 0.f && p->D == 64 && p->F == 128 && tile_rows(ws) == 16 && !wave_tiles(p, ws) && !DR4SR_ENV("DR4SR_NO_FUSE")
           && A.row_keep != nullptr;
}

template <int BM>
static int post_launch_bm(const dr4sr_sasrec_plan* p, const Workspace& ws, const PostArgs& A, bool bwd, hipStream_t s) {
    dim3 grid((ws.Tmax + BM - 1) / BM), blk(256);
    if (A.xcd) grid.x = xcd_grid((int)grid.x, BM);
    const size_t lds = (BM == 16 && A.at.on) ? sizeof(float) * att_lds_off(p->D, p->F) + att_lds_bytes(p->D) : post_lds(p->D, p->F, BM);
    if constexpr (BM == 16) {
        if (row_keep_saved(p, ws, A)) {
            if (bwd && A.at.kv_part) { big_lds((k_post_bwd<16, 64, 128, false, true, true>), lds); hipLaunchKernelGGL((k_post_bwd<16, 64, 128, false, true, true>), grid, blk, lds, s, A); }
            else if (bwd) { big_lds((k_post_bwd<16, 64, 128, false, false, true>), lds); hipLaunchKernelGGL((k_post_bwd<16, 64, 128, false, false, true>), grid, blk, lds, s, A); }
// ... 940 lines not shown
```

dr4sr_amd/csrc/prep_body.h:

```cpp
#pragma once
#include "common.h"

#define DR4SR_TINY_MAX 8

struct PermSel { const int64_t* perm; int64_t n, stride, offset; int* counter; };

struct PrepArgs {
    const int64_t* seqlen; const int64_t* rows; int* cu; int* state; int B, L, bump_rng; PermSel sel; int* tile_seq; int* seq_class;
    int* len_buf;
};

#define PREP_MAX_BLK 1024
__device__ __forceinline__ int prep_clamp_len(int64_t n, int L) { return (int)(n < 0 ? 0 : (n > L ? L : n)); }
__device__ __forceinline__ void prep_pub(unsigned long long* p, unsigned long long v) { __hip_atomic_store(p, v, __ATOMIC_RELAXED, __HIP_MEMORY_SCOPE_AGENT); }
__device__ __forceinline__ unsigned long long prep_get(const unsigned long long* p) { return __hip_atomic_load(p, __ATOMIC_RELAXED, __HIP_MEMORY_SCOPE_AGENT); }

template <int NT>
__device__ __forceinline__ void prep_scan2(unsigned long long s, unsigned long long s2, unsigned long long* part,
                                           unsigned long long& ex, unsigned long long& ex2, unsigned long long& tot, unsigned long long& tot2) {
    constexpr int NWV = NT / 64;
    const int lane = threadIdx.x & 63, wv = threadIdx.x >> 6;
    unsigned long long inc = s, inc2 = s2;
#pragma unroll
    for (int o = 1; o < 64; o <<= 1) {
        const unsigned long long v = __shfl_up(inc, o, 64), v2 = __shfl_up(inc2, o, 64);
        if (lane >= o) { inc += v; inc2 += v2; }
    }
    if (lane == 63) { part[wv] = inc; part[NWV + wv] = inc2; }
    __syncthreads();
    unsigned long long before = 0, before2 = 0;
    tot = 0; tot2 = 0;
#pragma unroll
    for (int w = 0; w < NWV; ++w) {
        const unsigned long long v = part[w], v2 = part[NWV + w];
        before += w < wv ? v : 0ull; before2 += w < wv ? v2 : 0ull;
        tot += v; tot2 += v2;
    }
    ex = before + inc - s; ex2 = before2 + inc2 - s2;
    __syncthreads();
}

template <int NT>
__device__ __forceinline__ void prep_phase1(const PrepArgs& P, const int blk, const int nblk, unsigned long long* part) {
    const PermSel sel = P.sel;
    const int64_t c = sel.perm ? (int64_t)*sel.counter : 0;
    int64_t* rw = const_cast<int64_t*>(P.rows);
    const int B = P.B, C = (B + nblk - 1) / nblk, b_lo = min(B, blk * C), b_hi = min(B, b_lo + C);
    unsigned long long* pre = reinterpret_cast<unsigned long long*>(P.len_buf);
    unsigned long long carry = 0, carry2 = 0;
    for (int c0 = b_lo; c0 < b_hi; c0 += NT) {
        const int b = c0 + threadIdx.x;
        int nn = 0;
        if (b < b_hi) {
            int64_t row = b;
            if (sel.perm) { row = sel.perm[(c * sel.stride + sel.offset + b) % sel.n]; __hip_atomic_store(rw + b, row, __ATOMIC_RELAXED, __HIP_MEMORY_SCOPE_AGENT); }
            else if (P.rows) row = P.rows[b];
            nn = prep_clamp_len(P.seqlen[row], P.L);
        }
        const unsigned long long s = (unsigned long long)nn + (nn > DR4SR_TINY_MAX && nn <= 16 ? (1ull << 32) : 0ull);
        const unsigned long long s2 = (nn > 16 ? 1ull : 0ull) + (nn > 0 && nn <= DR4SR_TINY_MAX ? (1ull << 32) : 0ull);
        unsigned long long ex, ex2, tot, tot2;
        prep_scan2<NT>(s, s2, part, ex, ex2, tot, tot2);
        if (b < b_hi) {
            prep_pub(pre + 2 * (size_t)b, carry + ex);
            prep_pub(pre + 2 * (size_t)b + 1, ((carry2 + ex2) & 0xffffffffull) | ((unsigned long long)(((carry2 + ex2) >> 32) & 0xffffu) << 32)
                                                  | ((unsigned long long)nn << 48));
        }
        carry += tot; carry2 += tot2;
    }
    if (threadIdx.x == 0) { prep_pub(pre + 2 * (size_t)(B + blk), carry); prep_pub(pre + 2 * (size_t)(B + blk) + 1, carry2); }
}

template <int NT>
__device__ __forceinline__ void prep_phase2(const PrepArgs& P, const int nblk, unsigned long long* part, int4* boff, const int wg = 0,
                                            const int nwg = 1) {
    const int B = P.B, C = (B + nblk - 1) / nblk;
    const unsigned long long* pre = reinterpret_cast<const unsigned long long*>(P.len_buf);
    int* __restrict__ cu = P.cu; int* __restrict__ tile_seq = P.tile_seq; int* __restrict__ seq_class = P.seq_class;
    const int64_t* rw = P.rows;
    unsigned long long carry = 0, carry2 = 0;
    for (int k0 = 0; k0 < nblk; k0 += NT) {
        const int k = k0 + threadIdx.x;
        unsigned long long s = 0, s2 = 0;
        if (k < nblk) { s = prep_get(pre + 2 * (size_t)(B + k)); s2 = prep_get(pre + 2 * (size_t)(B + k) + 1); }
        unsigned long long ex, ex2, tot, tot2;
        prep_scan2<NT>(s, s2, part, ex, ex2, tot, tot2);
        if (k < nblk) {
            const unsigned long long a = carry + ex, a2 = carry2 + ex2;
            boff[k] = make_int4((int)(a & 0xffffffffull), (int)(a >> 32), (int)(a2 & 0xffffffffull), (int)(a2 >> 32));
        }
        carry += tot; carry2 += tot2;
    }
    __syncthreads();
    const bool need_row = seq_class != nullptr && (P.sel.perm || rw);
    constexpr int U = 8;
    for (int b0 = wg * U * NT + threadIdx.x; b0 < B; b0 += nwg * U * NT) {
        unsigned long long w0[U], w1[U]; int64_t rowv[U];
#pragma unroll
        for (int u = 0; u < U; ++u) {
            const int b = b0 + u * NT;
            w0[u] = 0; w1[u] = 0; rowv[u] = b;
            if (b < B) {
                w0[u] = prep_get(pre + 2 * (size_t)b); w1[u] = prep_get(pre + 2 * (size_t)b + 1);
                if (need_row) rowv[u] = __hip_atomic_load(const_cast<int64_t*>(rw) + b, __ATOMIC_RELAXED, __HIP_MEMORY_SCOPE_AGENT);
            }
        }
#pragma unroll
        for (int u = 0; u < U; ++u) {
            const int b = b0 + u * NT;
            if (b >= B) break;
            const int4 o = boff[b / C];
            const int run = o.x + (int)(w0[u] & 0xffffffffull), nn = (int)(w1[u] >> 48);
            cu[b] = run;
            if (tile_seq)
                for (int q = (run + 15) >> 4; (q << 4) < run + nn; ++q) tile_seq[q] = b;
            if (seq_class && nn > 0) {
                if (nn <= DR4SR_TINY_MAX) {
                    const int nt = o.w + (int)((w1[u] >> 32) & 0xffffu);
                    seq_class[4 + 6 * B + nt] = b;
                    reinterpret_cast<int4*>(seq_class + 4)[nt] = make_int4(run, nn, b, (int)rowv[u]);
                } else if (nn <= 16) seq_class[4 + 4 * B + o.y + (int)(w0[u] >> 32)] = b;
                else seq_class[4 + 5 * B + o.z + (int)(w1[u] & 0xffffffffull)] = b;
            }
        }
    }
    if (wg != 0) return;
    if (P.sel.perm && threadIdx.x == 0) *P.sel.counter = *P.sel.counter + 1;
    if (threadIdx.x == NT - 1) {
        const int T = (int)(carry & 0xffffffffull);
        cu[B] = T;
        P.state[DR4SR_STATE_T] = T;
        if (P.bump_rng) P.state[DR4SR_STATE_RNGSTEP] += 1;
        if (seq_class) { seq_class[0] = (int)(carry >> 32); seq_class[1] = (int)(carry2 & 0xffffffffull); seq_class[2] = (int)(carry2 >> 32); }
    }
}

template <int NT>
__device__ __forceinline__ void prep_body(const PrepArgs& P, unsigned long long* part) {
    const int64_t* __restrict__ seqlen = P.seqlen; const int64_t* rows = P.rows;
    int* __restrict__ cu = P.cu; int* __restrict__ state = P.state; const int B = P.B, L = P.L, bump_rng = P.bump_rng;
    const PermSel sel = P.sel; int* __restrict__ tile_seq = P.tile_seq; int* __restrict__ seq_class = P.seq_class;
    constexpr int KEEP = 8, NWV = NT / 64;
    const int tid = threadIdx.x, lane = tid & 63, wv = tid >> 6;
    const int64_t c = sel.perm ? (int64_t)*sel.counter : 0;
    int64_t* rw = const_cast<int64_t*>(rows);
    unsigned long long carry = 0;
    unsigned int carry2 = 0;
    const int kr = min(KEEP, (B + NT - 1) / NT);
    for (int chunk0 = 0; chunk0 < B; chunk0 += NT * kr) {
        const int b0 = chunk0 + tid * kr, b1 = min(B, b0 + kr);
        int keep[KEEP]; int64_t krow[KEEP];
#pragma unroll
        for (int k = 0; k < KEEP; ++k) {
            keep[k] = 0; krow[k] = 0;
            if (b0 + k < b1) {
                const int b = b0 + k;
                if (sel.perm) { krow[k] = sel.perm[(c * sel.stride + sel.offset + b) % sel.n]; rw[b] = krow[k]; }
                else krow[k] = rows ? rows[b] : (int64_t)b;
            }
        }
#pragma unroll
        for (int k = 0; k < KEEP; ++k) if (b0 + k < b1) keep[k] = prep_clamp_len(seqlen[krow[k]], L);
        unsigned long long s = 0;
        unsigned int s2 = 0;
#pragma unroll
        for (int k = 0; k < KEEP; ++k) {
            const int nn = keep[k];
            s += (unsigned long long)nn + (nn > DR4SR_TINY_MAX && nn <= 16 ? (1ull << 32) : 0ull) + (nn > 16 ? (1ull << 48) : 0ull);
            s2 += nn > 0 && nn <= DR4SR_TINY_MAX ? 1u : 0u;
        }
        unsigned long long inc = s;
        unsigned int inc2 = s2;
#pragma unroll
        for (int o = 1; o < 64; o <<= 1) {
            const unsigned long long v = __shfl_up(inc, o, 64);
            const unsigned int v2 = __shfl_up(inc2, o, 64);
            if (lane >= o) { inc += v; inc2 += v2; }
        }
        if (lane == 63) { part[wv] = inc; part[NWV + wv] = inc2; }
        __syncthreads();
        unsigned long long before = 0, tot = 0;
        unsigned int before2 = 0, tot2 = 0;
#pragma unroll
        for (int w = 0; w < NWV; ++w) {
            const unsigned long long v = part[w];
            const unsigned int v2 = (unsigned int)part[NWV + w];
            before += w < wv ? v : 0ull;
            before2 += w < wv ? v2 : 0u;
            tot += v;
            tot2 += v2;
        }
        const unsigned long long ex = carry + before + inc - s;
        int run = (int)(ex & 0xffffffffull), ns = (int)((ex >> 32) & 0xffff), nl = (int)(ex >> 48);
        int nt = (int)(carry2 + before2 + inc2 - s2);
#pragma unroll
        for (int k = 0; k < KEEP; ++k) {
            if (b0 + k < b1) {
                const int b = b0 + k, nn = keep[k];
                cu[b] = run;
                if (tile_seq)
                    for (int q = (run + 15) >> 4; (q << 4) < run + nn; ++q) tile_seq[q] = b;
                if (seq_class && nn > 0) {
                    if (nn <= DR4SR_TINY_MAX) {
                        seq_class[4 + 6 * B + nt] = b;
                        reinterpret_cast<int4*>(seq_class + 4)[nt] = make_int4(run, nn, b, (int)krow[k]);
                        ++nt;
                    } else if (nn <= 16) seq_class[4 + 4 * B + ns++] = b;
                    else seq_class[4 + 5 * B + nl++] = b;
                }
// ... 16 lines not shown
```

dr4sr_amd/csrc/step.hip:

```cpp
#include "common.h"
#include "kernels.h"

#include <atomic>
#include <cstdlib>
#include <mutex>
#include <unordered_map>
void big_lds_impl(const void* kernel, size_t bytes) {
    static std::unordered_map<const void*, size_t> granted;
    static std::mutex mu;
    std::lock_guard<std::mutex> lk(mu);
    size_t& g = granted[kernel];
    if (bytes > g) {
        (void)hipFuncSetAttribute(kernel, hipFuncAttributeMaxDynamicSharedMemorySize, (int)bytes);
        g = bytes;
    }
}

extern "C" int dr4sr_abi_version(void) { return DR4SR_ABI_VERSION; }

static StepFork g_fork = {};
const StepFork& step_fork() {
    if (g_fork.state == 0 && DR4SR_XENV("DR4SR_STREAMS")) {
        hipStreamCaptureMode mode = hipStreamCaptureModeRelaxed;
        (void)hipThreadExchangeStreamCaptureMode(&mode);
// ... 85 lines not shown
    return 0;
}

static bool det_kv_shape(const dr4sr_sasrec_plan* p) { return p->H == 2 && p->L <= 64 && (p->D == 64 || p->D == 128) && (int64_t)p->B * p->L <= 131072; }
static bool det_lat_capable(const dr4sr_sasrec_plan* p) { return attn_tile_capable(p) && det_kv_shape(p); }

int carve_workspace(const dr4sr_sasrec_plan* p, Workspace* ws) {
    const int64_t D = p->D, F = p->F, Tmax = (int64_t)p->B * p->L;
    ws->n_params = dr4sr_sasrec_param_layout(p->n_items, p->L, p->D, p->F, p->n_layer, ws->off);
    ws->Tmax = (int)Tmax;
    {
        const bool forced = DR4SR_XENV("DR4SR_LATENCY_TMAX") != nullptr;
        const int64_t hint = p->expected_tokens < Tmax ? p->expected_tokens : Tmax;
        const bool known = hint > 0 && !forced;
        const bool wave_capable = p->H == 2 && p->L <= 64 && !DR4SR_ENV("DR4SR_NO_FUSE") && !DR4SR_ENV("DR4SR_ATTN_LISTS") && !DR4SR_ENV("DR4SR_ATTN_NOSPLIT")
                                  && !DR4SR_ENV("DR4SR_ATTN_VALU");
        const bool short_plan = hint <= 16 * (int64_t)p->B;
        const int64_t scale_tokens = !attn_tile_capable(p) ? DR4SR_SCALE_TOKENS
                                     : (short_plan ? (wave_capable ? DR4SR_SCALE_TOKENS_SHORT_WAVE : DR4SR_SCALE_TOKENS_SHORT) : DR4SR_SCALE_TOKENS_LONG);
        ws->scale = known ? hint * D > scale_tokens * 64 : at_scale((int)Tmax);
        ws->attn_split = known ? (hint * D > (int64_t)(wave_capable ? (scale_tokens < DR4SR_ATTN_SPLIT_TOKENS ? scale_tokens : DR4SR_ATTN_SPLIT_TOKENS) : DR4SR_ATTN_SPLIT_TOKENS) * 64 && short_plan)
                               : at_scale((int)Tmax);
        ws->det = DR4SR_ENV("DR4SR_DETERMINISTIC") != nullptr && atoi(DR4SR_ENV("DR4SR_DETERMINISTIC")) != 0;
        ws->det_lat = false;
        if (ws->det) {
            ws->det_lat = !ws->scale && !ws->attn_split && det_lat_capable(p) && !DR4SR_XENV("DR4SR_DET_SCALE_FORMS");
            ws->scale = true;
            if (p->H == 2 && p->L <= 64 && !DR4SR_ENV("DR4SR_NO_FUSE")) ws->attn_split = true;
        }
        if (const char* f = DR4SR_ENV("DR4SR_FORCE_SCALE")) {
            ws->scale = ws->attn_split = atoi(f) != 0;
            if (ws->det) ws->det_lat = !ws->scale && det_lat_capable(p) && !DR4SR_XENV("DR4SR_DET_SCALE_FORMS");
        }
        if (const char* f = DR4SR_ENV("DR4SR_FORCE_ATTN_SPLIT")) { ws->attn_split = atoi(f) != 0; if (ws->attn_split) ws->det_lat = false; }
        ws->scale_wg = ws->scale || ws->det;
        if (ws->det_lat) { ws->scale = false; ws->attn_split = false; }
        else if (ws->det) ws->scale = true;
        ws->attn_tile_sa = DR4SR_XENV("DR4SR_ATTN_WINDOW") && ws->attn_split && p->D == 64 && hint > 0 && hint <= 16 * (int64_t)p->B
                           && attn_tile_capable(p) && !DR4SR_ENV("DR4SR_ATTN_NOSPLIT");
    }
    char* base = (char*)p->workspace;
    int64_t o = 0;
    auto take = [&](int64_t nfloat) -> float* {
        float* r = base ? (float*)(base + o) : nullptr;
        o += ((nfloat * 4 + 255) / 256) * 256;
        return r;
    };
    ws->cu = (int*)take(p->B + 1);
    ws->tile_seq = (int*)take((Tmax + 15) / 16 + 1);
    ws->seq_class = (int*)take(4 + 7LL * p->B);
    ws->len_buf = (int*)take(4 * (int64_t)p->B + 4 * PREP_MAX_BLK);
    ws->attn_rd = take(Tmax * p->H);
    for (int i = 0; i <= p->n_layer; ++i) { ws->X[i] = take(Tmax * D); ws->dX[i] = take(Tmax * D); }
    ws->dctx = take(Tmax * D);
    ws->de_rec = (int4*)take(Tmax * 4); ws->idx32 = (int*)take(Tmax); ws->tok = (int2*)take(2 * Tmax);
    ws->de_ent = (int4*)take(Tmax * 12); ws->de_off = (unsigned char*)take((Tmax / 16 + 1) * 257);
    ws->wT_stride = 4 * D * D + 2 * D * F;
    ws->wT = take(ws->wT_stride * p->n_layer);
    ws->det_stride = D == 64 ? 64 * 64 + 64 : (int64_t)(D > F ? D : F) * (D > F ? D : F) + (D > F ? D : F);
    ws->det_part = nullptr; ws->det_ln = nullptr; ws->det_dp = nullptr; ws->det_kv = nullptr;
    ws->det_kv_layer = ((Tmax + 15) / 16) * 5 * 16 * 2 * D;
    if (ws->det && det_kv_shape(p)) ws->det_kv = take(ws->det_kv_layer * p->n_layer);
    if (ws->det) {
        const int64_t det_jobs = D == 64 ? 4 + 2 * F / 64 : 6;
        ws->det_part = take((int64_t)p->n_layer * det_jobs * DR4SR_DET_MAX_SPLITS * ws->det_stride);
        ws->det_ln = take((int64_t)p->n_layer * DR4SR_DET_MAX_SPLITS * 4 * D);
        ws->det_dp = take((int64_t)DR4SR_DET_MAX_SPLITS * p->L * D);
    }
    ws->wfrag = D == 128 ? take(ws->wT_stride * p->n_layer) : nullptr;
    ws->wsplit_E = D == 128 ? ws->wT_stride : 0;
    ws->wsplit = ws->wsplit_E ? reinterpret_cast<unsigned short*>(take(2 * ws->wsplit_E * p->n_layer)) : nullptr;
    if (!base && ws->wsplit_E) ws->wsplit = reinterpret_cast<unsigned short*>(1);
    ws->score_part = take(2LL * (p->B > (Tmax + 15) / 16 ? p->B : (Tmax + 15) / 16));
    ws->ln_part = take((int64_t)p->n_layer * ((Tmax + 15) / 16) * 4 * D);
    for (int l = 0; l < p->n_layer; ++l) {
        LayerWs& w = ws->layer[l];
        w.qkv = take(Tmax * 3 * D); w.ctx = take(Tmax * D); w.attn_st = take(Tmax * p->H * 2);
        w.attn_keep = reinterpret_cast<unsigned*>(take(Tmax * p->H * 2));
        w.u1 = take(Tmax * D); w.y = take(Tmax * D); w.st1 = take(Tmax * 2);
        w.a = take(Tmax * F); w.h = take(Tmax * F); w.u2 = take(Tmax * D); w.st2 = take(Tmax * 2);
        w.df = take(Tmax * D); w.da = take(Tmax * F); w.du1 = take(Tmax * D); w.dout = take(Tmax * D); w.dqkv = take(Tmax * 3 * D);
    }
    for (int l = 0; l < p->n_layer; ++l) ws->layer[l].row_keep = reinterpret_cast<unsigned short*>(take(Tmax * 8));
    ws->bytes = o;
    return 0;
}

extern "C" int64_t dr4sr_sasrec_workspace_bytes(const dr4sr_sasrec_plan* plan) {
    if (!plan) return DR4SR_E_ARG;
    dr4sr_sasrec_plan q = *plan;
    q.workspace = nullptr;
    if (q.B <= 0 || q.L <= 0 || q.n_layer <= 0 || q.n_layer > DR4SR_MAX_LAYERS) return DR4SR_E_ARG;
    if (check_shape(&q)) return DR4SR_E_SHAPE;
    Workspace ws;
    carve_workspace(&q, &ws);
    return ws.bytes;
}

extern "C" int dr4sr_sasrec_at_scale(const dr4sr_sasrec_plan* plan) {
    if (!plan) return DR4SR_E_ARG;
    dr4sr_sasrec_plan q = *plan;
    q.workspace = nullptr;
    if (q.B <= 0 || q.L <= 0 || q.n_layer <= 0 || q.n_layer > DR4SR_MAX_LAYERS) return DR4SR_E_ARG;
    if (check_shape(&q)) return DR4SR_E_SHAPE;
    Workspace ws;
    carve_workspace(&q, &ws);
    return (ws.scale ? 1 : 0) | (ws.attn_split ? 2 : 0) | (attn_in_tile(&q, ws) ? 4 : 0) | (ws.attn_tile_sa ? 8 : 0) | (attn_wave_on(&q, ws) ? 16 : 0)
           | (attn_fold_fwd(&q, ws) ? 32 : 0) | (ws.det_lat ? 64 : 0);
}

static int get_ws(const dr4sr_sasrec_plan* p, Workspace* ws) {
    int rc = check_plan(p);
    if (rc) return rc;
    if (!p->workspace) return DR4SR_E_ARG;
    carve_workspace(p, ws);
    if (ws->bytes > p->workspace_bytes) return DR4SR_E_WS;
    return 0;
}

struct AdamNext { int enable; int phase2_launch; PrepArgs prep; };
template <int OPT>
__global__ __launch_bounds__(256) void k_adam(float* __restrict__ P, float* __restrict__ G, float* __restrict__ M,
                                              float* __restrict__ V, int64_t n, int* __restrict__ state, float lr, float b1,
                                              float b2, float eps, float wd, float* __restrict__ loss_log,
                                              const int* __restrict__ log_index, const AdamNext next) {
    __shared__ float sh[2];
    __shared__ unsigned long long part[256];
    __shared__ int4 boff[PREP_MAX_BLK];
    const int t = state[DR4SR_STATE_STEP] + 1;
    const float nvalid = G[n];
    const float gs = nvalid > 0.f ? 1.0f / nvalid : 0.f;
    const bool poisoned = G[n + 2] != 0.f;
    const int nblk = next.enable == 1 ? (int)gridDim.x - 1 : (int)gridDim.x, blk = next.enable == 1 ? (int)blockIdx.x - 1 : (int)blockIdx.x;
    if (next.enable == 2) {
        if (loss_log && blk == 0 && threadIdx.x == 0) loss_log[log_index ? max(*log_index - 1, 0) : 0] = G[n + 1] * gs;
        prep_phase1<256>(next.prep, blk, nblk, part);
    }
    if (blk < 0) {
        const float lossv = G[n + 1] * gs;
        if (loss_log && threadIdx.x == 0) loss_log[log_index ? max(*log_index - 1, 0) : 0] = lossv;
        __syncthreads();
        prep_body<256>(next.prep, part);
    } else {
        if (threadIdx.x == 0) {
            const double bc1 = 1.0 - pow((double)b1, (double)t), bc2 = 1.0 - pow((double)b2, (double)t);
            sh[0] = (float)((double)lr / bc1);
            sh[1] = (float)(1.0 / sqrt(bc2));
        }
        __syncthreads();
        const float step_size = sh[0], inv_sqrt_bc2 = sh[1];
        if (!next.enable && loss_log && blk == 0 && threadIdx.x == 0) loss_log[log_index ? max(*log_index - 1, 0) : 0] = G[n + 1] * gs;
        const int64_t n4 = n / 4;
        auto upd = [&](float& pe, float& me, float& ve, float ge) {
            const float g = ge * gs + wd * pe;
            if constexpr (OPT == DR4SR_OPT_SGD) {
                pe = pe - lr * g;
            } else if constexpr (OPT == DR4SR_OPT_ADAGRAD) {
                ve = ve + g * g;
                pe = pe - lr * (g / (sqrtf(ve) + eps));
            } else if constexpr (OPT == DR4SR_OPT_RMSPROP) {
                ve = ve * b2 + (1.0f - b2) * g * g;
                pe = pe - lr * (g / (sqrtf(ve) + eps));
            } else {
                me = me + (g - me) * (1.0f - b1);
                ve = ve * b2 + (1.0f - b2) * g * g;
                const float denom = sqrtf(ve) * inv_sqrt_bc2 + eps;
                pe = pe - step_size * (me / denom);
            }
        };
        constexpr bool useM = OPT == DR4SR_OPT_ADAM, useV = OPT != DR4SR_OPT_SGD;
        const int64_t stride = (int64_t)nblk * 256;
        const float4 z4 = make_float4(0.f, 0.f, 0.f, 0.f);
        for (int64_t i = (int64_t)blk * 256 + threadIdx.x; i < n4; i += 2 * stride) {
            const int64_t j = i + stride;
            const bool two = j < n4;
            if (poisoned) {
                if (next.enable) { st4(G + 4 * i, z4); if (two) st4(G + 4 * j, z4); }
                continue;
            }
            float4 p0 = ld4(P + 4 * i), m0 = useM ? ld4(M + 4 * i) : z4, v0 = useV ? ld4(V + 4 * i) : z4;
            const float4 g0 = ld4(G + 4 * i);
            float4 p1 = p0, m1 = m0, v1 = v0, g1 = g0;
            if (two) { p1 = ld4(P + 4 * j); if (useM) m1 = ld4(M + 4 * j); if (useV) v1 = ld4(V + 4 * j); g1 = ld4(G + 4 * j); }
            upd(p0.x, m0.x, v0.x, g0.x); upd(p0.y, m0.y, v0.y, g0.y); upd(p0.z, m0.z, v0.z, g0.z); upd(p0.w, m0.w, v0.w, g0.w);
            st4(P + 4 * i, p0); if (useM) st4(M + 4 * i, m0); if (useV) st4(V + 4 * i, v0);
            if (next.enable) st4(G + 4 * i, z4);
            if (two) {
                upd(p1.x, m1.x, v1.x, g1.x); upd(p1.y, m1.y, v1.y, g1.y); upd(p1.z, m1.z, v1.z, g1.z); upd(p1.w, m1.w, v1.w, g1.w);
                st4(P + 4 * j, p1); if (useM) st4(M + 4 * j, m1); if (useV) st4(V + 4 * j, v1);
                if (next.enable) st4(G + 4 * j, z4);
            }
        }
    }
    __shared__ int s_last;
    if (next.enable == 2) asm volatile("s_waitcnt vmcnt(0)" ::: "memory");
    __syncthreads();
    if (threadIdx.x == 0) {
        const int ticket = atomicAdd(&state[8], 1);
        s_last = ticket == (int)gridDim.x - 1;
        if (s_last) {
            state[8] = 0;
            if (!poisoned) state[DR4SR_STATE_STEP] = t;
            if (next.enable) { G[n] = 0.f; G[n + 1] = 0.f; G[n + 2] = 0.f; G[n + 3] = 0.f; }
        }
    }
    if (next.enable == 2 && !next.phase2_launch) {
        __syncthreads();
        if (s_last) prep_phase2<256>(next.prep, (int)gridDim.x, part, boff);
    }
}

__global__ __launch_bounds__(256) void k_prep_phase2(const PrepArgs P, const int nblk) {
    __shared__ unsigned long long part[256];
    __shared__ int4 boff[PREP_MAX_BLK];
    prep_phase2<256>(P, nblk, part, boff, (int)blockIdx.x, (int)gridDim.x);
}

int launch_adam_flat(float* P, float* G, float* M, float* V, int64_t n, int* state, float lr, float b1, float b2,
                     float eps, float wd, hipStream_t s, float* loss_log, const int* log_index, const PrepArgs* next, int opt) {
    if (!P || !G || !M || !V || !state || n <= 0 || (n & 3) || opt < DR4SR_OPT_ADAM || opt > DR4SR_OPT_RMSPROP) return DR4SR_E_ARG;
    int64_t blocks = (n / 4 + 255) / 256;
    const int cap = DR4SR_ENV("DR4SR_ADAM_BLOCKS") ? atoi(DR4SR_ENV("DR4SR_ADAM_BLOCKS")) : 256;
    if (blocks > cap) blocks = cap;
    AdamNext nx;
    nx.enable = next ? (next->B > 1024 && next->len_buf && blocks <= PREP_MAX_BLK && (next->B + blocks - 1) / blocks < 65536 ? 2 : 1) : 0;
    nx.phase2_launch = 0;
    if (next) nx.prep = *next; else nx.prep = PrepArgs{nullptr, nullptr, nullptr, nullptr, 0, 0, 0, PermSel{nullptr, 0, 0, 0, nullptr}, nullptr, nullptr, nullptr};
    const bool p2_inline = DR4SR_ENV("DR4SR_PREP2_INLINE") != nullptr;
    nx.phase2_launch = nx.enable == 2 && !p2_inline;
    const dim3 grid((unsigned)blocks + (nx.enable == 1 ? 1 : 0));
    switch (opt) {
        case DR4SR_OPT_SGD: hipLaunchKernelGGL(k_adam<DR4SR_OPT_SGD>, grid, dim3(256), 0, s, P, G, M, V, n, state, lr, b1, b2, eps, wd, loss_log, log_index, nx); break;
        case DR4SR_OPT_ADAGRAD: hipLaunchKernelGGL(k_adam<DR4SR_OPT_ADAGRAD>, grid, dim3(256), 0, s, P, G, M, V, n, state, lr, b1, b2, eps, wd, loss_log, log_index, nx); break;
        case DR4SR_OPT_RMSPROP: hipLaunchKernelGGL(k_adam<DR4SR_OPT_RMSPROP>, grid, dim3(256), 0, s, P, G, M, V, n, state, lr, b1, b2, eps, wd, loss_log, log_index, nx); break;
        default: hipLaunchKernelGGL(k_adam<DR4SR_OPT_ADAM>, grid, dim3(256), 0, s, P, G, M, V, n, state, lr, b1, b2, eps, wd, loss_log, log_index, nx);
    }
    if (nx.phase2_launch) {
        const int B = next->B, per = 8 * 256;
        int g2 = (B + per - 1) / per;
        if (g2 > 256) g2 = 256;
        hipLaunchKernelGGL(k_prep_phase2, dim3(g2), dim3(256), 0, s, nx.prep, (int)blocks);
    }
    return DR4SR_LAUNCH_CHECK();
}
int launch_adam(const dr4sr_sasrec_plan* p, hipStream_t s, const PrepArgs* next) {
    return launch_adam_flat(p->params, p->grads, p->adam_m, p->adam_v, p->n_params, p->state, p->lr, p->beta1, p->beta2,
                            p->adam_eps, p->weight_decay, s, p->loss_log, p->perm ? p->perm_counter : nullptr, next, p->optimizer);
}

extern "C" int dr4sr_adam_step(const dr4sr_sasrec_plan* plan, void* stream) {
    if (!plan || plan->abi_version != DR4SR_ABI_VERSION || !plan->params || !plan->state) return DR4SR_E_ARG;
    return launch_adam(plan, (hipStream_t)stream);
}

__global__ __launch_bounds__(256) void k_zero(float* __restrict__ p, int64_t n4) {
    for (int64_t i = (int64_t)blockIdx.x * 256 + threadIdx.x; i < n4; i += (int64_t)gridDim.x * 256)
        st4(p + 4 * i, make_float4(0.f, 0.f, 0.f, 0.f));
}
static int launch_zero_grads(const dr4sr_sasrec_plan* p, int64_t n_params, hipStream_t s) {
    const int64_t n4 = (n_params + DR4SR_GRAD_TAIL) / 4;
    int64_t blocks = (n4 + 255) / 256;
    if (blocks > 512) blocks = 512;
    hipLaunchKernelGGL(k_zero, dim3((unsigned)blocks), dim3(256), 0, s, p->grads, n4);
    return DR4SR_LAUNCH_CHECK();
}

#define RC(x) do { int _rc = (x); if (_rc) return _rc; } while (0)

static bool use_mfma_attn(const dr4sr_sasrec_plan* p) {
    const bool off = DR4SR_ENV("DR4SR_ATTN_VALU") != nullptr;
    return p->H == 2 && (!off || !valu_attn_fits(p));
}
static int attn_fwd(const dr4sr_sasrec_plan* p, const Workspace& ws, int l, int training, hipStream_t s) {
    if (ws.attn_tile_sa) return launch_attn_tile_fwd(p, ws, l, training, s);
    return use_mfma_attn(p) ? launch_attn2_fwd(p, ws, l, training, s) : launch_attn_fwd(p, ws, l, training, s);
}
static int attn_bwd(const dr4sr_sasrec_plan* p, const Workspace& ws, int l, int training, hipStream_t s) {
    if (ws.attn_tile_sa) return launch_attn_tile_bwd(p, ws, l, training, s);
    return use_mfma_attn(p) ? launch_attn2_bwd(p, ws, l, training, s) : launch_attn_bwd(p, ws, l, training, s);
}

static int forward_layers(const dr4sr_sasrec_plan* p, const Workspace& ws, int training, hipStream_t s, bool mid_fused = false) {
    const bool fuse = DR4SR_ENV("DR4SR_NO_FUSE") == nullptr;
    if (tile_bf3(p, ws)) RC(launch_wsplit(p, ws, s));
    if (fuse) RC(launch_embqkv_fwd(p, ws, training, s));
    else { RC(launch_embed_fwd(p, ws, training, s)); if (wfrag_img_on(p, ws)) RC(launch_wfrag_write(p, ws, s)); }
    const bool in_tile = attn_in_tile(p, ws);
    for (int l = 0; l < p->n_layer; ++l) {
        if (!fuse) RC(launch_qkv_fwd(p, ws, l, s));
        if (!in_tile && !attn_fold_fwd(p, ws)) RC(attn_fwd(p, ws, l, training, s));
        if (!(mid_fused && l == p->n_layer - 1)) RC(launch_post_fwd(p, ws, l, training, s));
    }
    return 0;
}

static int dp_split_layer(const dr4sr_sasrec_plan* p) {
    int v = p->n_layer / 2 > 1 ? p->n_layer / 2 : 1;
    if (const char* e = DR4SR_ENV("DR4SR_DP_SPLIT_LAYER")) v = atoi(e);
    return v < 0 ? 0 : (v > p->n_layer ? p->n_layer : v);
}
static bool dp_two_buckets(const dr4sr_sasrec_plan* p, const Workspace& ws) {
    return !DR4SR_ENV("DR4SR_NO_FUSE") && !step_fork().on() && wgrad_table_jobs(p, ws) && dp_split_layer(p) > 0;
}

static int backward_layers(const dr4sr_sasrec_plan* p, const Workspace& ws, int training, int with_score, hipStream_t s,
                           bool mid_fused = false, bool meta = false, int phase = 0) {
    const bool fused = !DR4SR_ENV("DR4SR_NO_FUSE");
    const bool two = phase != 0 && dp_two_buckets(p, ws);
    if (phase == 2) return two ? launch_wgrad(p, ws, training, with_score, s, fused, meta, 0, dp_split_layer(p), 0) : 0;
    const StepFork& fk = step_fork();
    const bool early = fused && fk.on() && p->n_layer > 1 && !DR4SR_XENV("DR4SR_WGRAD_ONE_LAUNCH");
    bool forked = false;
    for (int l = p->n_layer - 1; l >= 0; --l) {
        if (!(mid_fused && l == p->n_layer - 1)) RC(launch_post_bwd(p, ws, l, training, s));
        if (!attn_in_tile(p, ws)) RC(attn_bwd(p, ws, l, training, s));
        if (!fused) RC(launch_qkv_bwd(p, ws, l, s));
        if (early && l >= 1) {
            RC(fk.fork(s, 2, 1));
            RC(launch_wgrad(p, ws, training, with_score, fk.side(s, 2), true, meta, l, l + 1));
            forked = true;
        }
    }
    if (!fused) RC(launch_embed_bwd(p, ws, training, s));
    else if (!qeb_in_wgrad(ws)) RC(launch_qkv_embed_bwd(p, ws, training, s));
// ... 20 lines not shown

extern "C" int dr4sr_sasrec_fwd_bwd(const dr4sr_sasrec_plan* plan, void* stream) {
    Workspace ws;
    RC(get_ws(plan, &ws));
    if (!plan->grads || !plan->item_id || !plan->neg_item || plan->n_params != ws.n_params) return DR4SR_E_ARG;
    hipStream_t s = (hipStream_t)stream;
    RC(launch_prep(plan, ws, 1, 1, s));
    return fwd_bwd_core(plan, ws, s);
}

static int fwd_bwd_weighted(const dr4sr_sasrec_plan* plan, const dr4sr_meta_weighting* mw, void* stream, bool prepared) {
    Workspace ws;
    RC(get_ws(plan, &ws));
    if (!mw || !mw->phi || !(mw->tau > 0.f) || !plan->grads || !plan->item_id || !plan->neg_item || plan->n_params != ws.n_params)
        return DR4SR_E_ARG;
    if (plan->D != 64) return DR4SR_E_SHAPE;
    hipStream_t s = (hipStream_t)stream;
    if (!prepared) RC(launch_prep(plan, ws, 1, 1, s));
    RC(forward_layers(plan, ws, 1, s, true));
    RC(launch_post_mid(plan, ws, 1, s, mw));
    RC(backward_layers(plan, ws, 1, 2, s, true, true));
    return 0;
}
extern "C" int dr4sr_sasrec_fwd_bwd_weighted(const dr4sr_sasrec_plan* plan, const dr4sr_meta_weighting* mw, void* stream) {
    return fwd_bwd_weighted(plan, mw, stream, false);
}
extern "C" int dr4sr_sasrec_fwd_bwd_weighted_prepared(const dr4sr_sasrec_plan* plan, const dr4sr_meta_weighting* mw, void* stream) {
    return fwd_bwd_weighted(plan, mw, stream, true);
}

extern "C" int dr4sr_sasrec_train_step(const dr4sr_sasrec_plan* plan, void* stream) {
    RC(dr4sr_sasrec_fwd_bwd(plan, stream));
    return dr4sr_adam_step(plan, stream);
}

extern "C" int dr4sr_sasrec_fwd_bwd_prepared(const dr4sr_sasrec_plan* plan, void* stream) {
    Workspace ws;
    RC(get_ws(plan, &ws));
    if (!plan->grads || !plan->item_id || !plan->neg_item || plan->n_params != ws.n_params) return DR4SR_E_ARG;
    return fwd_bwd_core(plan, ws, (hipStream_t)stream);
}
extern "C" int dr4sr_sasrec_grad_buckets(const dr4sr_sasrec_plan* plan, int64_t* bounds) {
    if (!plan) return DR4SR_E_ARG;
    dr4sr_sasrec_plan q = *plan;
    q.workspace = nullptr;
    if (q.B <= 0 || q.L <= 0 || q.n_layer <= 0 || q.n_layer > DR4SR_MAX_LAYERS) return DR4SR_E_ARG;
    if (check_shape(&q)) return DR4SR_E_SHAPE;
    Workspace ws;
    carve_workspace(&q, &ws);
    const bool two = dp_two_buckets(&q, ws);
    if (bounds) {
        bounds[0] = 0;
        bounds[1] = two ? ws.off[2] : ws.n_params + DR4SR_GRAD_TAIL;
        bounds[2] = ws.n_params + DR4SR_GRAD_TAIL;
    }
    return two ? 2 : 1;
}
extern "C" int dr4sr_sasrec_fwd_bwd_phase(const dr4sr_sasrec_plan* plan, int32_t prepared, int32_t phase, void* stream) {
    Workspace ws;
    RC(get_ws(plan, &ws));
    if (phase < 1 || phase > 2 || !plan->grads || !plan->item_id || !plan->neg_item || plan->n_params != ws.n_params) return DR4SR_E_ARG;
    hipStream_t s = (hipStream_t)stream;
    if (phase == 1 && !prepared) RC(launch_prep(plan, ws, 1, 1, s));
    return fwd_bwd_core(plan, ws, s, phase);
}
extern "C" int dr4sr_adam_step_prepare_next(const dr4sr_sasrec_plan* plan, void* stream) {
    Workspace ws;
    RC(get_ws(plan, &ws));
    if (!plan->grads || plan->n_params != ws.n_params) return DR4SR_E_ARG;
    PrepArgs next;
    RC(make_prep_args(plan, ws, 1, &next));
    return launch_adam(plan, (hipStream_t)stream, &next);
}

extern "C" int dr4sr_sasrec_train_steps(const dr4sr_sasrec_plan* plan, int32_t n_steps, void* stream) {
    Workspace ws;
    RC(get_ws(plan, &ws));
    if (n_steps <= 0 || !plan->grads || !plan->item_id || !plan->neg_item || plan->n_params != ws.n_params) return DR4SR_E_ARG;
    const bool nofuse_env = DR4SR_ENV("DR4SR_NO_PREP_FUSE") != nullptr;
    const bool nofuse = nofuse_env;
    hipStream_t s = (hipStream_t)stream;
    PrepArgs next;
    RC(make_prep_args(plan, ws, 1, &next));
    RC(launch_prep(plan, ws, 1, 1, s));
    for (int i = 0; i < n_steps; ++i) {
        RC(fwd_bwd_core(plan, ws, s));
        const bool last = i == n_steps - 1;
        if (nofuse && !last) { RC(launch_adam(plan, s)); RC(launch_prep(plan, ws, 1, 1, s)); }
        else RC(launch_adam(plan, s, last ? nullptr : &next));
    }
    return 0;
}

extern "C" int dr4sr_sasrec_encode(const dr4sr_sasrec_plan* plan, int32_t training, int32_t pooling, float* out,
                                   void* stream) {
    Workspace ws;
    RC(get_ws(plan, &ws));
    if (!out || pooling < DR4SR_POOL_NONE || pooling > DR4SR_POOL_MEAN) return DR4SR_E_ARG;
    hipStream_t s = (hipStream_t)stream;
    RC(launch_prep(plan, ws, training ? 1 : 0, 0, s));
    RC(forward_layers(plan, ws, training, s));
    return launch_unpack(plan, ws, ws.X[plan->n_layer], out, pooling == DR4SR_POOL_LAST ? 1 : pooling == DR4SR_POOL_MEAN ? 2 : 0, s);
}

extern "C" int dr4sr_sasrec_encode_bwd(const dr4sr_sasrec_plan* plan, int32_t training, int32_t pooling,
                                       const float* d_out, void* stream) {
    Workspace ws;
    RC(get_ws(plan, &ws));
    if (!d_out || !plan->grads || pooling < DR4SR_POOL_NONE || pooling > DR4SR_POOL_MEAN) return DR4SR_E_ARG;
    hipStream_t s = (hipStream_t)stream;
    RC(launch_pack(plan, ws, d_out, ws.dX[plan->n_layer], pooling == DR4SR_POOL_LAST ? 1 : pooling == DR4SR_POOL_MEAN ? 2 : 0, s));
    return backward_layers(plan, ws, training, 0, s);
}

extern "C" int dr4sr_sasrec_launch_kernel(const dr4sr_sasrec_plan* plan, int32_t kernel, int32_t layer, void* stream) {
    return dr4sr_sasrec_launch_kernel_weighted(plan, nullptr, kernel, layer, stream);
}
extern "C" int dr4sr_sasrec_launch_kernel_weighted(const dr4sr_sasrec_plan* plan, const dr4sr_meta_weighting* mw, int32_t kernel,
                                                   int32_t layer, void* stream) {
    Workspace ws;
    RC(get_ws(plan, &ws));
    if (layer < 0 || layer >= plan->n_layer) return DR4SR_E_ARG;
    hipStream_t s = (hipStream_t)stream;
    switch (kernel) {
        case DR4SR_K_PREP: return launch_prep(plan, ws, 0, 0, s);
        case DR4SR_K_EMBED_FWD: return launch_embed_fwd(plan, ws, 1, s);
        case DR4SR_K_QKV_FWD: return launch_qkv_fwd(plan, ws, layer, s);
        case DR4SR_K_ATTN_FWD: return attn_fwd(plan, ws, layer, 1, s);
        case DR4SR_K_POST_FWD: return launch_post_fwd(plan, ws, layer, 1, s);
        case DR4SR_K_SCORE: return launch_score_packed(plan, ws, s);
        case DR4SR_K_TRANSPOSE: return launch_transpose_weights(plan, ws, s);
        case DR4SR_K_POST_BWD: return launch_post_bwd(plan, ws, layer, 1, s);
        case DR4SR_K_ATTN_BWD: return attn_bwd(plan, ws, layer, 1, s);
        case DR4SR_K_QKV_BWD: return launch_qkv_bwd(plan, ws, layer, s);
        case DR4SR_K_EMBED_BWD: return launch_embed_bwd(plan, ws, 1, s);
        case DR4SR_K_WGRAD: return launch_wgrad(plan, ws, 1, 1, s);
        case DR4SR_K_ADAM: return launch_adam(plan, s);
        case DR4SR_K_ZERO_GRADS: return launch_zero_grads(plan, ws.n_params, s);
        case DR4SR_K_EMBQKV_FWD: return launch_embqkv_fwd(plan, ws, 1, s);
        case DR4SR_K_POST_MID: return launch_post_mid(plan, ws, 1, s, mw);
        case DR4SR_K_QKV_EMBED_BWD: return launch_qkv_embed_bwd(plan, ws, 1, s);
        case DR4SR_K_WGRAD_FUSED: return launch_wgrad(plan, ws, 1, 2, s, true, mw != nullptr);
        default: return DR4SR_E_ARG;
    }
}
```

include/dr4sr_hip.h:

```cpp
#ifndef DR4SR_HIP_H
#define DR4SR_HIP_H

#include <stdint.h>

#ifdef __cplusplus
extern "C" {
#endif

#define DR4SR_ABI_VERSION 10

#define DR4SR_E_ARG      (-1)
#define DR4SR_E_SHAPE    (-2)
#define DR4SR_E_WS       (-3)
#define DR4SR_E_RCCL_BASE (-100)

#define DR4SR_SITE_EMB   0
#define DR4SR_SITE_ATTN  1
#define DR4SR_SITE_PROJ  2
#define DR4SR_SITE_ACT   3
#define DR4SR_SITE_FFN   4

#define DR4SR_OPT_ADAM    0
#define DR4SR_OPT_SGD     1
#define DR4SR_OPT_ADAGRAD 2
#define DR4SR_OPT_RMSPROP 3

#define DR4SR_POOL_NONE   0
#define DR4SR_POOL_ORIGIN 1
#define DR4SR_POOL_LAST   2
#define DR4SR_POOL_MEAN   3

#define DR4SR_STATE_STEP     0
#define DR4SR_STATE_T        1
#define DR4SR_STATE_NVALID   2
#define DR4SR_STATE_RNGSTEP  3
#define DR4SR_STATE_WORDS    16

#define DR4SR_GRAD_TAIL 4

typedef struct dr4sr_sasrec_plan {
    int32_t abi_version;
    int32_t B, L, D, H, F, n_layer, n_items;
    float   ln_eps;
    float   p_drop;
    uint64_t seed;
    float*  params;
    float*  grads;
    float*  adam_m;
    float*  adam_v;
    int64_t n_params;
    const int64_t* in_item_id;
    const int64_t* item_id;
    const int64_t* seqlen;
    const int64_t* rows;
    int64_t* neg_item;
    int32_t  sample_neg;
    void*    workspace;
    int64_t  workspace_bytes;
    int32_t* state;
    float lr, beta1, beta2, adam_eps, weight_decay;
    const int64_t* perm;
    int64_t  n_perm;
    int64_t  perm_stride;
    int64_t  perm_offset;
    int32_t* perm_counter;
    float*   loss_log;
    int32_t  expected_tokens;
    int32_t  optimizer;
} dr4sr_sasrec_plan;

int  dr4sr_abi_version(void);
int  dr4sr_sasrec_plan_sizeof(void);
int64_t dr4sr_sasrec_param_layout(int32_t n_items, int32_t L, int32_t D, int32_t F, int32_t n_layer,
                                  int64_t* offsets );
int64_t dr4sr_sasrec_workspace_bytes(const dr4sr_sasrec_plan* plan);
int dr4sr_sasrec_at_scale(const dr4sr_sasrec_plan* plan);


int dr4sr_sasrec_fwd_bwd(const dr4sr_sasrec_plan* plan, void* stream);

int dr4sr_adam_step(const dr4sr_sasrec_plan* plan, void* stream);

int dr4sr_sasrec_train_step(const dr4sr_sasrec_plan* plan, void* stream);

int dr4sr_sasrec_train_steps(const dr4sr_sasrec_plan* plan, int32_t n_steps, void* stream);

int dr4sr_sasrec_fwd_bwd_prepared(const dr4sr_sasrec_plan* plan, void* stream);
int dr4sr_adam_step_prepare_next(const dr4sr_sasrec_plan* plan, void* stream);

int dr4sr_sasrec_grad_buckets(const dr4sr_sasrec_plan* plan, int64_t* bounds );
int dr4sr_sasrec_fwd_bwd_phase(const dr4sr_sasrec_plan* plan, int32_t prepared, int32_t phase, void* stream);

#define DR4SR_COMM_ID_BYTES 128
#define DR4SR_RED_SUM 0
#define DR4SR_RED_MAX 1
#define DR4SR_RED_MIN 2
typedef struct dr4sr_comm dr4sr_comm;
int dr4sr_comm_unique_id(void* id_out );
int dr4sr_comm_init_rank(const void* id , int32_t rank, int32_t world, int32_t device, dr4sr_comm** out);
int dr4sr_comm_destroy(dr4sr_comm* comm);
int dr4sr_comm_rank(const dr4sr_comm* comm);
int dr4sr_comm_world(const dr4sr_comm* comm);
int dr4sr_comm_async_error(dr4sr_comm* comm);
const char* dr4sr_comm_error_string(int rc);
int dr4sr_allreduce_f32(dr4sr_comm* comm, float* buf, int64_t n, void* stream);
int dr4sr_allreduce_f64(dr4sr_comm* comm, double* buf, int64_t n, int32_t op , void* stream);
int dr4sr_allreduce_f32_async(dr4sr_comm* comm, float* buf, int64_t n, void* stream);
int dr4sr_comm_join(dr4sr_comm* comm, void* stream);
int dr4sr_allgather_bytes(dr4sr_comm* comm, const void* send, void* recv , int64_t bytes, void* stream);
int dr4sr_broadcast_bytes(dr4sr_comm* comm, void* buf, int64_t bytes, int32_t root, void* stream);

int dr4sr_sasrec_encode(const dr4sr_sasrec_plan* plan, int32_t training, int32_t pooling,
                        float* out, void* stream);
int dr4sr_sasrec_encode_bwd(const dr4sr_sasrec_plan* plan, int32_t training, int32_t pooling,
                            const float* d_out, void* stream);

int dr4sr_select_rows(const int64_t* perm, int64_t n_perm, int64_t* rows_out, int32_t B,
                      int64_t stride, int64_t offset, int32_t* counter, void* stream);

int dr4sr_embed_gather_posadd(const float* E, const float* P, const int64_t* idx, float* out,
                              int64_t B, int32_t L, int32_t D, int32_t n_items, void* stream);

int dr4sr_score_bce_fwd(const float* query, const float* E, const int64_t* target,
                        const int64_t* neg, float* pos_score, float* neg_score, float* loss_pos,
                        float* stats, int64_t B, int32_t L, int32_t D, void* stream);
int dr4sr_score_bce_bwd(const float* query, const float* E, const int64_t* target,
                        const int64_t* neg, const float* w, const float* scale, float* d_query,
                        float* dE, int64_t B, int32_t L, int32_t D, void* stream);

int dr4sr_score_bpr_fwd(const float* query, const float* E, const int64_t* target,
                        const int64_t* neg, float* pos_score, float* neg_score, float* loss_pos,
                        float* stats, int64_t B, int32_t L, int32_t D, void* stream);
int dr4sr_score_bpr_bwd(const float* query, const float* E, const int64_t* target,
                        const int64_t* neg, const float* w, const float* scale, float* d_query,
                        float* dE, int64_t B, int32_t L, int32_t D, void* stream);
int dr4sr_loss_from_scores_fwd(const float* pos, const float* neg, int64_t n, int32_t K, int32_t kind, float* loss_pos,
                               float* stats, void* stream);
int dr4sr_loss_from_scores_bwd(const float* pos, const float* neg, int64_t n, int32_t K, int32_t kind, const float* g,
                               const float* scale, float* d_pos, float* d_neg, void* stream);

int dr4sr_neg_sample(int64_t* out, int64_t n, int32_t n_items, uint64_t seed, uint32_t step,
                     void* stream);
int dr4sr_neg_sample_dev(int64_t* out, int64_t n, int32_t n_items, uint64_t seed, const int32_t* step_dev, void* stream);

int dr4sr_check_ids(const int64_t* idx, int64_t n, int32_t n_items, int32_t* bad_count, void* stream);

int dr4sr_full_score_topk(const float* q, const float* E, const int64_t* hist, float* out_score,
                          int64_t* out_item, int64_t B, int32_t D, int32_t n_items, int32_t Lh,
                          int32_t k, void* stream);
int64_t dr4sr_full_score_topk_workspace_bytes(int64_t B, int32_t n_items);
int dr4sr_full_score_topk_ws(const float* q, const float* E, const int64_t* hist, float* out_score, int64_t* out_item, int64_t B,
                             int32_t D, int32_t n_items, int32_t Lh, int32_t k, float* workspace, int64_t workspace_bytes,
                             void* stream);

int dr4sr_full_score_topk_masked_ws(const float* q, const float* E, const int64_t* hist, const uint8_t* item_blocked,
                                    float* out_score, int64_t* out_item, int64_t B, int32_t D, int32_t n_items, int32_t Lh,
                                    int32_t k, float* workspace, int64_t workspace_bytes, void* stream);

// ... 229 lines not shown
```

Baseline: 2.668 million sequences/s.

## Skip dead LN/activation stores, cache attention keep bits, precompute Adam bias terms

In the fused post-attention forward with a carried row state, the LayerNorm pre-activation, row-stat and FFN pre-activation stores are compiled out and their pointers nulled, since backward recomputes them from carried state. Attention dropout keep bits are stored in forward and reloaded in backward instead of regenerating RNG. Adam bias-correction terms are computed once in the prep kernel into a two-slot record keyed by step and hyperparameters, so each Adam block reads them without a pow/sqrt and a block barrier. The cost is extra workspace, a small keep-bit buffer and more template variants, and correctness depends on no remaining consumer needing the dropped tensors.

```diff
diff --git a/dr4sr_amd/_lib.py b/dr4sr_amd/_lib.py
--- a/dr4sr_amd/_lib.py
+++ b/dr4sr_amd/_lib.py
@@ -127,6 +127,7 @@
     "dr4sr_sasrec_plan_sizeof": (C.c_int, []),
     "dr4sr_sasrec_param_layout": (C.c_int64, [C.c_int32, C.c_int32, C.c_int32, C.c_int32, C.c_int32, C.c_void_p]),
     "dr4sr_sasrec_workspace_bytes": (C.c_int64, [_PLANP]),
+    "dr4sr_sasrec_workspace_offsets": (C.c_int, [_PLANP, C.c_int32, C.POINTER(C.c_int64)]),
     "dr4sr_sasrec_at_scale": (C.c_int, [C.c_void_p]),
     "dr4sr_sasrec_fwd_bwd": (C.c_int, [_PLANP, C.c_void_p]),
     "dr4sr_adam_step": (C.c_int, [_PLANP, C.c_void_p]),
diff --git a/dr4sr_amd/csrc/attn_tile.h b/dr4sr_amd/csrc/attn_tile.h
--- a/dr4sr_amd/csrc/attn_tile.h
+++ b/dr4sr_amd/csrc/attn_tile.h
@@ -159,6 +159,16 @@
         const RngKey rk = make_rng(P.seed, (uint32_t)P.state[DR4SR_STATE_RNGSTEP], P.p);
         keep_bits(rk, DR4SR_SITE_ATTN + 4 * P.layer, ((uint64_t)((mq.y & 0xfffff) * 2 + h) * 64 + i) * 64, i, k.lo, k.hi);
     }
+    return k;
+}
+__device__ __forceinline__ void keep_store(const TileAttnArgs& A, const Keep k, const int t0, const int T) {
+    const int lane = threadIdx.x & 63, w = threadIdx.x >> 6, tq = t0 + lane;
+    if (w < 2 && lane < 16 && tq < T) *reinterpret_cast<uint2*>(A.keep + ((size_t)tq * 2 + w) * 2) = make_uint2(k.lo, k.hi);
+}
+__device__ __forceinline__ Keep keep_load(const TileAttnArgs& A, const int t0, const int T) {
+    const int tq = t0 + (int)(threadIdx.x & 15), h = (threadIdx.x >> 6) & 1;
+    Keep k{0xffffffffu, 0xffffffffu};
+    if (tq < T) { const uint2 v = *reinterpret_cast<const uint2*>(A.keep + ((size_t)tq * 2 + h) * 2); k.lo = v.x; k.hi = v.y; }
     return k;
 }
 
diff --git a/dr4sr_amd/csrc/embed.hip b/dr4sr_amd/csrc/embed.hip
--- a/dr4sr_amd/csrc/embed.hip
+++ b/dr4sr_amd/csrc/embed.hip
@@ -63,14 +63,16 @@
     }
     __shared__ unsigned long long part[1024];
     prep_body<1024>(P, part);
+    if (P.bc_rec && threadIdx.x == 64) adam_bc_write(P.bc_rec, P.state[DR4SR_STATE_STEP] + 1, P.lr, P.b1, P.b2);
 }
 
 static int launch_prep_sel(const int64_t* seqlen, const int64_t* rows, int* cu, int* state, int B, int L, int bump_rng, float* zero,
-                           int64_t zero_floats, const PermSel& sel, int* tile_seq, int* seq_class, hipStream_t s) {
+                           int64_t zero_floats, const PermSel& sel, int* tile_seq, int* seq_class, hipStream_t s, const PrepArgs* bc = nullptr) {
     const int64_t n4 = zero ? zero_floats / 4 : 0;
     int zb = (int)((n4 + 1023) / 1024);
     if (zb > 255) zb = 255;
-    const PrepArgs P{seqlen, rows, cu, state, B, L, bump_rng, sel, tile_seq, seq_class, nullptr};
+    const PrepArgs P{seqlen, rows, cu, state, B, L, bump_rng, sel, tile_seq, seq_class, nullptr, bc ? bc->bc_rec : nullptr, bc ? bc->lr : 0.f,
+                     bc ? bc->b1 : 0.f, bc ? bc->b2 : 0.f};
     hipLaunchKernelGGL(k_prep, dim3(1 + zb), dim3(1024), 0, s, P, zero, n4);
     return DR4SR_LAUNCH_CHECK();
 }
@@ -88,15 +90,17 @@
         if (!p->rows || !p->perm_counter || p->n_perm <= 0) return DR4SR_E_ARG;
         sel = PermSel{p->perm, p->n_perm, p->perm_stride, p->perm_offset, p->perm_counter};
     }
-    *out = PrepArgs{p->seqlen, p->rows, ws.cu, p->state, p->B, p->L, bump_rng, sel, ws.tile_seq, (ws.attn_split && !attn_wave_on(p, ws)) ? ws.seq_class : nullptr, ws.len_buf};
+    int* bc_rec = (bump_rng && p->optimizer == DR4SR_OPT_ADAM && p->workspace) ? ws.bc_rec : nullptr;
+    *out = PrepArgs{p->seqlen, p->rows, ws.cu, p->state, p->B, p->L, bump_rng, sel, ws.tile_seq, (ws.attn_split && !attn_wave_on(p, ws)) ? ws.seq_class : nullptr, ws.len_buf,
+                    bc_rec, p->lr, p->beta1, p->beta2};
     return 0;
 }
-int launch_prep(const dr4sr_sasrec_plan* p, const Workspace& ws, int bump_rng, int zero_grads, hipStream_t s) {
+int launch_prep(const dr4sr_sasrec_plan* p, const Workspace& ws, int bump_rng, int zero_grads, hipStream_t s, int adam_bc) {
     PrepArgs P;
     const int rc = make_prep_args(p, ws, bump_rng, &P);
     if (rc) return rc;
     return launch_prep_sel(p->seqlen, p->rows, ws.cu, p->state, p->B, p->L, bump_rng, zero_grads ? p->grads : nullptr,
-                           ws.n_params + DR4SR_GRAD_TAIL, P.sel, ws.tile_seq, P.seq_class, s);
+                           ws.n_params + DR4SR_GRAD_TAIL, P.sel, ws.tile_seq, P.seq_class, s, adam_bc ? &P : nullptr);
 }
 
 
diff --git a/dr4sr_amd/csrc/kernels.h b/dr4sr_amd/csrc/kernels.h
--- a/dr4sr_amd/csrc/kernels.h
+++ b/dr4sr_amd/csrc/kernels.h
@@ -35,6 +35,7 @@
     bool scale, attn_split;
     bool attn_tile_sa;
     int* len_buf;
+    int* bc_rec;
     int* seq_class;
     float* attn_rd;
     int* tile_seq;
@@ -187,7 +188,7 @@
 
 int carve_workspace(const dr4sr_sasrec_plan* p, Workspace* ws);
 
-int launch_prep(const dr4sr_sasrec_plan* p, const Workspace& ws, int bump_rng, int zero_grads, hipStream_t s);
+int launch_prep(const dr4sr_sasrec_plan* p, const Workspace& ws, int bump_rng, int zero_grads, hipStream_t s, int adam_bc = 0);
 int make_prep_args(const dr4sr_sasrec_plan* p, const Workspace& ws, int bump_rng, PrepArgs* out);
 int launch_embed_fwd(const dr4sr_sasrec_plan* p, const Workspace& ws, int training, hipStream_t s);
 int launch_embed_bwd(const dr4sr_sasrec_plan* p, const Workspace& ws, int training, hipStream_t s);
diff --git a/dr4sr_amd/csrc/linear.hip b/dr4sr_amd/csrc/linear.hip
--- a/dr4sr_amd/csrc/linear.hip
+++ b/dr4sr_amd/csrc/linear.hip
@@ -293,7 +293,7 @@
     return make_float4((bits & 1u) ? k.scale : 0.f, (bits & 2u) ? k.scale : 0.f, (bits & 4u) ? k.scale : 0.f, (bits & 8u) ? k.scale : 0.f);
 }
 
-template <int BM, int D, bool RES_IN_LDS, bool COPY_LDS, bool CARRY = false, bool KPRE = false>
+template <int BM, int D, bool RES_IN_LDS, bool COPY_LDS, bool CARRY = false, bool KPRE = false, bool NOST = false>
 __device__ __forceinline__ void ln_rowpass(const float* __restrict__ Cs, int ldc, const float* res, int ldres,
                                            const float* __restrict__ lnw, const float* __restrict__ lnb, float eps,
                                            float* __restrict__ U, float* __restrict__ OUT, float* __restrict__ ST,
@@ -302,6 +302,7 @@
     constexpr int NV = D / 64, PASSES = BM / 16;
     static_assert(!CARRY || (NV == 1 && PASSES == 1), "the carried row state is one float4 per thread");
     static_assert(!KPRE || CARRY, "the keep bits arrive in the carried row state");
+    static_assert(!NOST || CARRY, "the row state leaves through *cy only");
     const int l16 = threadIdx.x & 15, rsub = threadIdx.x >> 4;
     float4 gam[NV], bet[NV], v[PASSES][NV];
     float mean[PASSES], rstd[PASSES];
@@ -326,7 +327,7 @@
                 if constexpr (CARRY && !KPRE) cy->keep = keep_bits4(m);
             }
             v[ps][j] = make_float4(r.x + o.x, r.y + o.y, r.z + o.z, r.w + o.w);
-            if (ok) st4(U + (size_t)t * D + c, v[ps][j]);
+            if constexpr (!NOST) { if (ok) st4(U + (size_t)t * D + c, v[ps][j]); }
         }
     }
 #pragma unroll
@@ -346,7 +347,7 @@
             if (yreg) yreg[ps][j] = ok ? yv : make_float4(0.f, 0.f, 0.f, 0.f);
             if (COPY_LDS) st4(Ls + row * ldl + c, ok ? yv : make_float4(0.f, 0.f, 0.f, 0.f));
         }
-        if (ok && l16 == 0) { ST[2 * (size_t)t] = mean[ps]; ST[2 * (size_t)t + 1] = rstd[ps]; }
+        if constexpr (!NOST) { if (ok && l16 == 0) { ST[2 * (size_t)t] = mean[ps]; ST[2 * (size_t)t + 1] = rstd[ps]; } }
     }
 }
 
@@ -387,6 +388,7 @@
     WFragT<PF ? D : 16, PF ? 3 * D : 64> f_nx;
     STAMP(0);
     static_assert(!KU || (BM == 16 && D == 64 && F == 128 && !FFN_ONLY && CARRY != 0), "one row, one float4, 16 keep bits per thread");
+    constexpr bool NOST = CARRY == 1;
     auto keep_upfront = [&]() {
         if constexpr (KU) {
             const uint32_t w = row_keep_word(rk, sP, sF, sA, actdrop, t0 + rsub);
@@ -426,6 +428,7 @@
                 __builtin_amdgcn_sched_barrier(0);
                 const tattn::Keep k = tattn::fwd_compute<D, KEEPQ>(A, t0, T, R0, LD, smem + att_lds_off(D, F), att_pre);
                 if (keep_out) *keep_out = k;
+                if constexpr (CARRY == 2) tattn::keep_store(A.at, k, t0, T);
                 __builtin_amdgcn_sched_barrier(0);
                 if (A.nx_qkv) { if constexpr (D == 128) wfrag_load_img(f_nx, reinterpret_cast<const float*>(A.sp) + WSplitGeo<D, F>::E); else wfrag_load(f_nx, A.nx_in_w, D); }
             } else {
@@ -450,6 +453,7 @@
                     tattn::fwd_stage<D, KEEPQ>(A, t0, T, smem + att_lds_off(D, F), att_pre);
                     const tattn::Keep k = tattn::fwd_compute<D, KEEPQ>(A, t0, T, R0, LD, smem + att_lds_off(D, F), att_pre);
                     if (keep_out) *keep_out = k;
+                    if constexpr (CARRY == 2) tattn::keep_store(A.at, k, t0, T);
                 }
             }
         }
@@ -463,7 +467,7 @@
         }
         lds_barrier(); STAMP(2);
         if constexpr (KU && !KU_EARLY) keep_upfront();
-        ln_rowpass<BM, D, false, true, CARRY != 0, KU>(R2, LD, A.x, D, A.ln1_w, A.ln1_b, A.eps, A.u1, A.y, A.st1, R1, LD, t0, T, dodrop, rk, sP, nullptr,
+        ln_rowpass<BM, D, false, true, CARRY != 0, KU, NOST>(R2, LD, A.x, D, A.ln1_w, A.ln1_b, A.eps, A.u1, A.y, A.st1, R1, LD, t0, T, dodrop, rk, sP, nullptr,
                                                   CARRY ? &cy->ln1 : nullptr);
     }
     lds_barrier(); STAMP(3);
@@ -497,7 +501,7 @@
                     h.x *= m.x; h.y *= m.y; h.z *= m.z; h.w *= m.w;
                     if constexpr (CARRY != 0 && !KU) cy->akeep |= keep_bits4(m) << (4 * j);
                 }
-                if (ok) { st4(A.a + (size_t)t * F + c, a4); st4(A.h + (size_t)t * F + c, h); }
+                if (ok) { if constexpr (!NOST) st4(A.a + (size_t)t * F + c, a4); st4(A.h + (size_t)t * F + c, h); }
                 st4(R2 + row * LF + c, h);
             }
         }
@@ -512,7 +516,7 @@
     }
     lds_barrier(); STAMP(6);
     if (!FFN_ONLY && A.nx_qkv) {
-        ln_rowpass<BM, D, true, true, CARRY != 0, KU>(R0, LD, R1, LD, A.ln2_w, A.ln2_b, A.eps, A.u2, A.z, A.st2, R1, LD, t0, T, dodrop, rk, sF, nullptr,
+        ln_rowpass<BM, D, true, true, CARRY != 0, KU, NOST>(R0, LD, R1, LD, A.ln2_w, A.ln2_b, A.eps, A.u2, A.z, A.st2, R1, LD, t0, T, dodrop, rk, sF, nullptr,
                                                   CARRY ? &cy->ln2 : nullptr);
         if constexpr (CARRY == 2) row_keep_store<F>(A, *cy, t0, T);
         lds_barrier();
@@ -523,7 +527,7 @@
         tile_to_global<BM, 3 * D>(acc, A.nx_qkv, 3 * D, A.nx_in_b, t0, T);
         if (A.nx_dqkv_zero) zero_kv_rows<BM, D>(A.nx_dqkv_zero, t0, T);
     } else {
-        ln_rowpass<BM, D, true, false, CARRY != 0, KU>(R0, LD, R1, LD, A.ln2_w, A.ln2_b, A.eps, A.u2, A.z, A.st2, nullptr, 0, t0, T, dodrop, rk, sF, zreg,
+        ln_rowpass<BM, D, true, false, CARRY != 0, KU, NOST>(R0, LD, R1, LD, A.ln2_w, A.ln2_b, A.eps, A.u2, A.z, A.st2, nullptr, 0, t0, T, dodrop, rk, sF, zreg,
                                                    CARRY ? &cy->ln2 : nullptr);
         if constexpr (CARRY == 2) row_keep_store<F>(A, *cy, t0, T);
     }
@@ -692,15 +696,21 @@
             if constexpr (CARRY == 3) {
                 const uint32_t w = ok ? (uint32_t)A.row_keep[16 * (size_t)t + l16] : 0u;
                 cy_ld.ln1.keep = w & 15u; cy_ld.ln2.keep = (w >> 4) & 15u; cy_ld.akeep = w >> 8;
+                if (at_stage) keep = tattn::keep_load(A.at, t0, T);
             }
             __builtin_amdgcn_sched_barrier(0);
         }
         if (at_stage) {
-            const int2 mq = tattn::own_word(A.at, t0, T);
-            att_st.issue(A.at, t0, T, (A.at.on & 4) ? tattn::NEAR0 : 0, tattn::WR);
-            __builtin_amdgcn_sched_barrier(0);
-            keep = tattn::own_keep(A, mq, t0, T);
-            __builtin_amdgcn_sched_barrier(0);
+            if constexpr (CARRY == 3) {
+                att_st.issue(A.at, t0, T, (A.at.on & 4) ? tattn::NEAR0 : 0, tattn::WR);
+                __builtin_amdgcn_sched_barrier(0);
+            } else {
+                const int2 mq = tattn::own_word(A.at, t0, T);
+                att_st.issue(A.at, t0, T, (A.at.on & 4) ? tattn::NEAR0 : 0, tattn::WR);
+                __builtin_amdgcn_sched_barrier(0);
+                keep = tattn::own_keep(A, mq, t0, T);
+                __builtin_amdgcn_sched_barrier(0);
+            }
         }
     }
     STAMP(16);
@@ -1256,6 +1266,7 @@
         if (!S.rec) Af.z = nullptr;
         tattn::Keep keep{0xffffffffu, 0xffffffffu};
         constexpr int CARRY = BM == 16 ? 1 : 0;
+        if constexpr (CARRY == 1) Af.u1 = Af.st1 = Af.a = Af.u2 = Af.st2 = nullptr;
         RowCarry<F> cy;
         post_fwd_body<BM, D, F, false, true, CARRY, KU>(Af, t0, T, zreg, &keep, &cy);
         if constexpr (BM != 16) score_prefetch<BM>(A, S, t0, T, P);
diff --git a/dr4sr_amd/csrc/prep_body.h b/dr4sr_amd/csrc/prep_body.h
--- a/dr4sr_amd/csrc/prep_body.h
+++ b/dr4sr_amd/csrc/prep_body.h
@@ -8,7 +8,23 @@
 struct PrepArgs {
     const int64_t* seqlen; const int64_t* rows; int* cu; int* state; int B, L, bump_rng; PermSel sel; int* tile_seq; int* seq_class;
     int* len_buf;
+    int* bc_rec;
+    float lr, b1, b2;
 };
+
+#define DR4SR_BC_SLOT_WORDS 8
+__device__ __forceinline__ void adam_bias_terms(const float lr, const float b1, const float b2, const int t, float& step_size, float& inv_sqrt_bc2) {
+    const double bc1 = 1.0 - pow((double)b1, (double)t), bc2 = 1.0 - pow((double)b2, (double)t);
+    step_size = (float)((double)lr / bc1);
+    inv_sqrt_bc2 = (float)(1.0 / sqrt(bc2));
+}
+__device__ __forceinline__ void adam_bc_write(int* rec, const int t, const float lr, const float b1, const float b2) {
+    float step_size, inv_sqrt_bc2;
+    adam_bias_terms(lr, b1, b2, t, step_size, inv_sqrt_bc2);
+    int* r = rec + DR4SR_BC_SLOT_WORDS * (t & 1);
+    *reinterpret_cast<int4*>(r) = make_int4(t, __float_as_int(lr), __float_as_int(b1), __float_as_int(b2));
+    *reinterpret_cast<int2*>(r + 4) = make_int2(__float_as_int(step_size), __float_as_int(inv_sqrt_bc2));
+}
 
 #define PREP_MAX_BLK 1024
 __device__ __forceinline__ int prep_clamp_len(int64_t n, int L) { return (int)(n < 0 ? 0 : (n > L ? L : n)); }
@@ -71,9 +87,9 @@
     if (threadIdx.x == 0) { prep_pub(pre + 2 * (size_t)(B + blk), carry); prep_pub(pre + 2 * (size_t)(B + blk) + 1, carry2); }
 }
 
-template <int NT>
+template <int NT, bool BCW = false>
 __device__ __forceinline__ void prep_phase2(const PrepArgs& P, const int nblk, unsigned long long* part, int4* boff, const int wg = 0,
-                                            const int nwg = 1) {
+                                            const int nwg = 1, const int t_next = -1) {
     const int B = P.B, C = (B + nblk - 1) / nblk;
     const unsigned long long* pre = reinterpret_cast<const unsigned long long*>(P.len_buf);
     int* __restrict__ cu = P.cu; int* __restrict__ tile_seq = P.tile_seq; int* __restrict__ seq_class = P.seq_class;
@@ -125,6 +141,7 @@
         }
     }
     if (wg != 0) return;
+    if constexpr (BCW) { if (threadIdx.x == 64) adam_bc_write(P.bc_rec, t_next >= 0 ? t_next : P.state[DR4SR_STATE_STEP] + 1, P.lr, P.b1, P.b2); }
     if (P.sel.perm && threadIdx.x == 0) *P.sel.counter = *P.sel.counter + 1;
     if (threadIdx.x == NT - 1) {
         const int T = (int)(carry & 0xffffffffull);
diff --git a/dr4sr_amd/csrc/step.hip b/dr4sr_amd/csrc/step.hip
--- a/dr4sr_amd/csrc/step.hip
+++ b/dr4sr_amd/csrc/step.hip
@@ -191,6 +191,7 @@
         w.df = take(Tmax * D); w.da = take(Tmax * F); w.du1 = take(Tmax * D); w.dout = take(Tmax * D); w.dqkv = take(Tmax * 3 * D);
     }
     for (int l = 0; l < p->n_layer; ++l) ws->layer[l].row_keep = reinterpret_cast<unsigned short*>(take(Tmax * 8));
+    ws->bc_rec = (int*)take(2 * DR4SR_BC_SLOT_WORDS);
     ws->bytes = o;
     return 0;
 }
@@ -206,6 +207,21 @@
     return ws.bytes;
 }
 
+extern "C" int dr4sr_sasrec_workspace_offsets(const dr4sr_sasrec_plan* plan, int32_t layer, int64_t* out) {
+    if (!plan || !out) return DR4SR_E_ARG;
+    dr4sr_sasrec_plan q = *plan;
+    if (q.B <= 0 || q.L <= 0 || q.n_layer <= 0 || q.n_layer > DR4SR_MAX_LAYERS || layer < 0 || layer >= q.n_layer) return DR4SR_E_ARG;
+    if (check_shape(&q)) return DR4SR_E_SHAPE;
+    char* const base = reinterpret_cast<char*>(uintptr_t(1) << 20);
+    q.workspace = base;
+    Workspace ws;
+    carve_workspace(&q, &ws);
+    const LayerWs& w = ws.layer[layer];
+    const void* const p[DR4SR_WS_OFF_COUNT] = {w.attn_keep, w.u1, w.st1, w.a, w.u2, w.st2, w.row_keep, ws.bc_rec};
+    for (int i = 0; i < DR4SR_WS_OFF_COUNT; ++i) out[i] = (int64_t)(reinterpret_cast<const char*>(p[i]) - base);
+    return 0;
+}
+
 extern "C" int dr4sr_sasrec_at_scale(const dr4sr_sasrec_plan* plan) {
     if (!plan) return DR4SR_E_ARG;
     dr4sr_sasrec_plan q = *plan;
@@ -228,7 +244,7 @@
 }
 
 struct AdamNext { int enable; int phase2_launch; PrepArgs prep; };
-template <int OPT>
+template <int OPT, bool BC = false>
 __global__ __launch_bounds__(256) void k_adam(float* __restrict__ P, float* __restrict__ G, float* __restrict__ M,
                                               float* __restrict__ V, int64_t n, int* __restrict__ state, float lr, float b1,
                                               float b2, float eps, float wd, float* __restrict__ loss_log,
@@ -237,6 +253,12 @@
     __shared__ unsigned long long part[256];
     __shared__ int4 boff[PREP_MAX_BLK];
     const int t = state[DR4SR_STATE_STEP] + 1;
+    int4 bk0, bk1; int2 bv0, bv1;
+    if constexpr (BC) {
+        const int* rec = next.prep.bc_rec;
+        bk0 = *reinterpret_cast<const int4*>(rec); bv0 = *reinterpret_cast<const int2*>(rec + 4);
+        bk1 = *reinterpret_cast<const int4*>(rec + DR4SR_BC_SLOT_WORDS); bv1 = *reinterpret_cast<const int2*>(rec + DR4SR_BC_SLOT_WORDS + 4);
+    }
     const float nvalid = G[n];
     const float gs = nvalid > 0.f ? 1.0f / nvalid : 0.f;
     const bool poisoned = G[n + 2] != 0.f;
@@ -250,14 +272,24 @@
         if (loss_log && threadIdx.x == 0) loss_log[log_index ? max(*log_index - 1, 0) : 0] = lossv;
         __syncthreads();
         prep_body<256>(next.prep, part);
+        if constexpr (BC) { if (threadIdx.x == 64) adam_bc_write(next.prep.bc_rec, poisoned ? t : t + 1, lr, b1, b2); }
     } else {
-        if (threadIdx.x == 0) {
-            const double bc1 = 1.0 - pow((double)b1, (double)t), bc2 = 1.0 - pow((double)b2, (double)t);
-            sh[0] = (float)((double)lr / bc1);
-            sh[1] = (float)(1.0 / sqrt(bc2));
+        float step_size, inv_sqrt_bc2;
+        if constexpr (BC) {
+            const int4 bk = (t & 1) ? bk1 : bk0;
+            const int2 bv = (t & 1) ? bv1 : bv0;
+            if (bk.x == t && bk.y == __float_as_int(lr) && bk.z == __float_as_int(b1) && bk.w == __float_as_int(b2)) {
+                step_size = __int_as_float(bv.x); inv_sqrt_bc2 = __int_as_float(bv.y);
+            } else adam_bias_terms(lr, b1, b2, t, step_size, inv_sqrt_bc2);
+        } else {
+            if (threadIdx.x == 0) {
+                const double bc1 = 1.0 - pow((double)b1, (double)t), bc2 = 1.0 - pow((double)b2, (double)t);
+                sh[0] = (float)((double)lr / bc1);
+                sh[1] = (float)(1.0 / sqrt(bc2));
+            }
+            __syncthreads();
+            step_size = sh[0]; inv_sqrt_bc2 = sh[1];
         }
-        __syncthreads();
-        const float step_size = sh[0], inv_sqrt_bc2 = sh[1];
         if (!next.enable && loss_log && blk == 0 && threadIdx.x == 0) loss_log[log_index ? max(*log_index - 1, 0) : 0] = G[n + 1] * gs;
         const int64_t n4 = n / 4;
         auto upd = [&](float& pe, float& me, float& ve, float ge) {
@@ -315,7 +347,7 @@
     }
     if (next.enable == 2 && !next.phase2_launch) {
         __syncthreads();
-        if (s_last) prep_phase2<256>(next.prep, (int)gridDim.x, part, boff);
+        if (s_last) prep_phase2<256, BC>(next.prep, (int)gridDim.x, part, boff, 0, 1, poisoned ? t : t + 1);
     }
 }
 
@@ -323,6 +355,11 @@
     __shared__ unsigned long long part[256];
     __shared__ int4 boff[PREP_MAX_BLK];
     prep_phase2<256>(P, nblk, part, boff, (int)blockIdx.x, (int)gridDim.x);
+}
+__global__ __launch_bounds__(256) void k_prep_phase2_bc(const PrepArgs P, const int nblk) {
+    __shared__ unsigned long long part[256];
+    __shared__ int4 boff[PREP_MAX_BLK];
+    prep_phase2<256, true>(P, nblk, part, boff, (int)blockIdx.x, (int)gridDim.x);
 }
 
 int launch_adam_flat(float* P, float* G, float* M, float* V, int64_t n, int* state, float lr, float b1, float b2,
@@ -334,7 +371,9 @@
     AdamNext nx;
     nx.enable = next ? (next->B > 1024 && next->len_buf && blocks <= PREP_MAX_BLK && (next->B + blocks - 1) / blocks < 65536 ? 2 : 1) : 0;
     nx.phase2_launch = 0;
-    if (next) nx.prep = *next; else nx.prep = PrepArgs{nullptr, nullptr, nullptr, nullptr, 0, 0, 0, PermSel{nullptr, 0, 0, 0, nullptr}, nullptr, nullptr, nullptr};
+    if (next) nx.prep = *next; else nx.prep = PrepArgs{nullptr, nullptr, nullptr, nullptr, 0, 0, 0, PermSel{nullptr, 0, 0, 0, nullptr}, nullptr, nullptr, nullptr, nullptr, 0.f, 0.f, 0.f};
+    if (opt != DR4SR_OPT_ADAM) nx.prep.bc_rec = nullptr;
+    else if (nx.prep.bc_rec) { nx.prep.lr = lr; nx.prep.b1 = b1; nx.prep.b2 = b2; }
     const bool p2_inline = DR4SR_ENV("DR4SR_PREP2_INLINE") != nullptr;
     nx.phase2_launch = nx.enable == 2 && !p2_inline;
     const dim3 grid((unsigned)blocks + (nx.enable == 1 ? 1 : 0));
@@ -342,13 +381,16 @@
         case DR4SR_OPT_SGD: hipLaunchKernelGGL(k_adam<DR4SR_OPT_SGD>, grid, dim3(256), 0, s, P, G, M, V, n, state, lr, b1, b2, eps, wd, loss_log, log_index, nx); break;
         case DR4SR_OPT_ADAGRAD: hipLaunchKernelGGL(k_adam<DR4SR_OPT_ADAGRAD>, grid, dim3(256), 0, s, P, G, M, V, n, state, lr, b1, b2, eps, wd, loss_log, log_index, nx); break;
         case DR4SR_OPT_RMSPROP: hipLaunchKernelGGL(k_adam<DR4SR_OPT_RMSPROP>, grid, dim3(256), 0, s, P, G, M, V, n, state, lr, b1, b2, eps, wd, loss_log, log_index, nx); break;
-        default: hipLaunchKernelGGL(k_adam<DR4SR_OPT_ADAM>, grid, dim3(256), 0, s, P, G, M, V, n, state, lr, b1, b2, eps, wd, loss_log, log_index, nx);
+        default:
+            if (next && next->bc_rec) hipLaunchKernelGGL((k_adam<DR4SR_OPT_ADAM, true>), grid, dim3(256), 0, s, P, G, M, V, n, state, lr, b1, b2, eps, wd, loss_log, log_index, nx);
+            else hipLaunchKernelGGL(k_adam<DR4SR_OPT_ADAM>, grid, dim3(256), 0, s, P, G, M, V, n, state, lr, b1, b2, eps, wd, loss_log, log_index, nx);
     }
     if (nx.phase2_launch) {
         const int B = next->B, per = 8 * 256;
         int g2 = (B + per - 1) / per;
         if (g2 > 256) g2 = 256;
-        hipLaunchKernelGGL(k_prep_phase2, dim3(g2), dim3(256), 0, s, nx.prep, (int)blocks);
+        if (nx.prep.bc_rec) hipLaunchKernelGGL(k_prep_phase2_bc, dim3(g2), dim3(256), 0, s, nx.prep, (int)blocks);
+        else hipLaunchKernelGGL(k_prep_phase2, dim3(g2), dim3(256), 0, s, nx.prep, (int)blocks);
     }
     return DR4SR_LAUNCH_CHECK();
 }
@@ -535,7 +577,7 @@
     hipStream_t s = (hipStream_t)stream;
     PrepArgs next;
     RC(make_prep_args(plan, ws, 1, &next));
-    RC(launch_prep(plan, ws, 1, 1, s));
+    RC(launch_prep(plan, ws, 1, 1, s, 1));
     for (int i = 0; i < n_steps; ++i) {
         RC(fwd_bwd_core(plan, ws, s));
         const bool last = i == n_steps - 1;
diff --git a/include/dr4sr_hip.h b/include/dr4sr_hip.h
--- a/include/dr4sr_hip.h
+++ b/include/dr4sr_hip.h
@@ -74,6 +74,16 @@
 int64_t dr4sr_sasrec_param_layout(int32_t n_items, int32_t L, int32_t D, int32_t F, int32_t n_layer,
                                   int64_t* offsets );
 int64_t dr4sr_sasrec_workspace_bytes(const dr4sr_sasrec_plan* plan);
+#define DR4SR_WS_OFF_ATTN_KEEP 0
+#define DR4SR_WS_OFF_U1        1
+#define DR4SR_WS_OFF_ST1       2
+#define DR4SR_WS_OFF_A         3
+#define DR4SR_WS_OFF_U2        4
+#define DR4SR_WS_OFF_ST2       5
+#define DR4SR_WS_OFF_ROW_KEEP  6
+#define DR4SR_WS_OFF_BC_REC    7
+#define DR4SR_WS_OFF_COUNT     8
+int dr4sr_sasrec_workspace_offsets(const dr4sr_sasrec_plan* plan, int32_t layer, int64_t* out);
 int dr4sr_sasrec_at_scale(const dr4sr_sasrec_plan* plan);
 
 
```

Result: faster. 2.742 million sequences/s, median of 6 (+2.8%).
